# corelab-src/dacapo

Hardware: AMD Instinct MI355X
Metric: NTT/s (NTT-equivalents over one run() of the ResNet HEVM program, nt=2^14) (higher is better)
Workload: dtype u64; 1 GPU; ResNet-20 (SiLU) HEVM program traced from the reference's examples/benchmarks/ResNet.py with its resnet20.silu.model weights, nt=2^14 slots, N=2^15, 14 x 60-bit primes (SEAL_HEVM.cpp:39-53); one independent ciphertext stream per GPU; streams_per_gpu=1, parallelism=replicas x1 (no collective in the op path)

## Files before the change

### dacapo_amd/csrc/batch_ops.hip

```cpp
#include <stdlib.h>

#include "galois.hpp"
#include "plan.hpp"

namespace dacapo {

constexpr int kBT = 256;

__global__ __launch_bounds__(kBT) void b_tensor_kernel(const MulItem *__restrict__ items, u64 *__restrict__ target, int ell,
                                                        size_t N, const DModulus *__restrict__ mods)
{
    const int i = blockIdx.y, b = blockIdx.z;
    const MulItem it = items[b];
    const DModulus m = mods[i];
    const size_t k = ((size_t)blockIdx.x * kBT + threadIdx.x) * 2;
    const u64x2 a0 = *reinterpret_cast<const u64x2 *>(it.a.limb(0, i, N) + k), a1 = *reinterpret_cast<const u64x2 *>(it.a.limb(1, i, N) + k);
    const u64x2 b0 = *reinterpret_cast<const u64x2 *>(it.b.limb(0, i, N) + k), b1 = *reinterpret_cast<const u64x2 *>(it.b.limb(1, i, N) + k);
    u64x2 c0, c1, c2;
#pragma unroll
    for (int e = 0; e < 2; e++) {
        c0[e] = mulmod(a0[e], b0[e], m);
        Acc128 acc;
        acc.clear();
        acc.mac(a0[e], b1[e]);
        acc.mac(a1[e], b0[e]);
        c1[e] = acc.reduce(m);
        c2[e] = mulmod(a1[e], b1[e], m);
    }
    *reinterpret_cast<u64x2 *>(it.dst.limb(0, i, N) + k) = c0;
    *reinterpret_cast<u64x2 *>(it.dst.limb(1, i, N) + k) = c1;
    const size_t o = ((size_t)b * ell + i) * N + k;
    *reinterpret_cast<u64x2 *>(target + o) = c2;
}

template <int MODE>
__global__ __launch_bounds__(kBT) void b_ks_mac_kernel(u64 *__restrict__ acc, const u64 *__restrict__ ext,
                                                        const u64 *__restrict__ target, const KsItem *__restrict__ items,
                                                        const u64 *__restrict__ shared_key, int ell, int K, size_t N, int logN,
                                                        const DModulus *__restrict__ mods)
{
    const int m = blockIdx.y, b = blockIdx.z, sp = K - 1;
    const int pm = (m == ell) ? sp : m;
    const DModulus M = mods[pm];
    const u64 *key = MODE == 0 ? items[b].key : shared_key;
    const u64 *tg = MODE == 0 ? nullptr : target + (size_t)b * ell * N;
    const u64 *ex = ext + (size_t)b * ell * ell * N;
    const size_t k = ((size_t)blockIdx.x * kBT + threadIdx.x) * 2;
    Acc128 a0[2], a1[2];
    u64 r0[2] = { 0, 0 }, r1[2] = { 0, 0 };
#pragma unroll
    for (int e = 0; e < 2; e++) a0[e].clear(), a1[e].clear();
    for (int j = 0; j < ell; j++) {
        u64x2 x;
        if (j == m && MODE == 0) {
            const u32 g = galois_idx((u32)k, items[b].elt, logN);
            const u64x2 v = *reinterpret_cast<const u64x2 *>(items[b].src.limb(1, j, N) + (g & ~1u));
            x = (g & 1u) ? u64x2{ v.y, v.x } : v;
        } else {
            const u64 *op = (j == m) ? tg + (size_t)j * N : ex + ((size_t)j * ell + (m < j ? m : m - 1)) * N;
            x = *reinterpret_cast<const u64x2 *>(op + k);
        }
        const u64x2 y0 = *reinterpret_cast<const u64x2 *>(key + (((size_t)j * 2 + 0) * K + pm) * N + k);
        const u64x2 y1 = *reinterpret_cast<const u64x2 *>(key + (((size_t)j * 2 + 1) * K + pm) * N + k);
#pragma unroll
        for (int e = 0; e < 2; e++) {
            a0[e].mac(x[e], y0[e]);
            a1[e].mac(x[e], y1[e]);
        }
        if ((j & 15) == 15) {
#pragma unroll
            for (int e = 0; e < 2; e++) {
                r0[e] = addmod(r0[e], a0[e].reduce(M), M.q);
                r1[e] = addmod(r1[e], a1[e].reduce(M), M.q);
                a0[e].clear(), a1[e].clear();
            }
        }
    }
    u64x2 o0, o1;
#pragma unroll
    for (int e = 0; e < 2; e++) {
        o0[e] = addmod(r0[e], a0[e].reduce(M), M.q);
        o1[e] = addmod(r1[e], a1[e].reduce(M), M.q);
    }
    u64 *ac = acc + (size_t)b * 2 * (ell + 1) * N;
    *reinterpret_cast<u64x2 *>(ac + ((size_t)0 * (ell + 1) + m) * N + k) = o0;
    *reinterpret_cast<u64x2 *>(ac + ((size_t)1 * (ell + 1) + m) * N + k) = o1;
}

static bool fuse_mac() { return option(OPT_KS_FUSE_MAC) != 0; }
static long big_threshold() { return (long)option(OPT_KS_BIG_TILES); }
static long fuse_mac_threshold() { return (long)option(OPT_KS_FUSE_MAC_TILES); }

bool chain_fusion_supported() { return fuse_mac() && fuse_mac_threshold() == (1L << 40); }

template <int MODE>
static void b_ks_tail(Context &c, const BatchWs &w, u64 *digits, const KsItem *items, const void *final_items, const u64 *shared_key, int B,
                      int ell, hipStream_t s, const Handoff &h)
{
    const size_t N = c.N;
    const int K = c.K, sp = K - 1;
    const long tiles = (long)(N >> 10) * B * ell * ell;
    const bool big = tiles >= big_threshold(), fused_mac = fuse_mac() && tiles < fuse_mac_threshold();
    if (big) {
        launch_ntt_cols_inv(c, digits, (long)N, B * ell, nullptr, 0, ell, s);
        f_ks_lift_fcols(c, digits, w.ext, B, ell, s);
    } else
        f_ks_icols_lift_fcols(c, digits, w.ext, B, ell, s);
    u64 *acc_last = w.acc + (size_t)ell * N;
    const long acc_ps = (long)(ell + 1) * (long)N;
    if (!fused_mac) {
        launch_ntt_rows_fwd(c, w.ext, (long)N, B * ell * ell, c.ks_prime_idx(ell), 0, ell * ell, s);
        DC_LAUNCH(b_ks_mac_kernel<MODE>, dim3((unsigned)(N / (2 * kBT)), ell + 1, B), dim3(kBT), 0, s, w.acc, w.ext, w.target, items,
                           shared_key, ell, K, N, c.logN, c.d_mods);
        f_irows_strided(c, acc_last, acc_ps, sp, 1, acc_last, acc_ps, 2 * B, s);
    } else
        f_ks_frows_mac(c, MODE, w.ext, MODE == 1 ? nullptr : w.target, MODE == 1 ? reinterpret_cast<const KsItem *>(final_items) : items,
                       shared_key, w.acc, B, ell, s, MODE == 0);
    if (big) {
        launch_ntt_cols_inv(c, acc_last, acc_ps, 2 * B, nullptr, sp, 1, s);
        f_dr_lift_fcols(c, acc_last, acc_ps, w.tmp, 2 * B, ell, sp, s);
    } else
        f_dr_icols_lift_fcols(c, acc_last, acc_ps, w.tmp, 2 * B, ell, sp, s);
    f_frows_final(c, (MODE == 1 && fused_mac) ? 4 : MODE, w.tmp, final_items, w.acc, 2 * B, ell, sp, s, RsItem{}, nullptr, nullptr, h,
                  MODE == 0 && fused_mac);
}

void b_rotate_hops(Context &c, const BatchWs &w, const KsItem *d_items, int B, int ell, hipStream_t s, const Handoff &h, int unique)
{
    if (c.hybrid()) {
        hyb_rotate_hops(c, w, d_items, B, ell, s, unique);
        return;
    }
    f_irows_rot_c1(c, d_items, ell, w.digits, B, s);
    b_ks_tail<0>(c, w, w.digits, d_items, d_items, nullptr, B, ell, s, h);
}

void b_mul_relin(Context &c, const BatchWs &w, const MulItem *d_items, const u64 *relin_key, int B, int ell, hipStream_t s, const Handoff &h)
{
    if (c.hybrid()) {
        hyb_mul_relin(c, w, d_items, relin_key, B, ell, s);
        return;
    }
    const size_t N = c.N;
    const bool fused_mac = fuse_mac() && (long)(N >> 10) * B * ell * ell < fuse_mac_threshold();
    u64 *digits = w.digits;
    if (h.in)
        digits = const_cast<u64 *>(h.in);
    else if (!fused_mac) {
        DC_LAUNCH(b_tensor_kernel, dim3((unsigned)(N / (2 * kBT)), ell, B), dim3(kBT), 0, s, d_items, w.target, ell, N, c.d_mods);
        f_irows_strided(c, w.target, (long)N, 0, ell, w.digits, (long)N, B * ell, s);
    } else
        f_irows_tensor_c2(c, d_items, ell, w.digits, B, s);
    b_ks_tail<1>(c, w, digits, nullptr, d_items, relin_key, B, ell, s, h);
}

bool mul_relin_rescale_fused(const Context &c, int B, int ell)
{
    const long tiles = (long)(c.N >> 10) * B * ell * ell;
    return !c.hybrid() && ell >= 2 && fuse_mac() && tiles < fuse_mac_threshold() && tiles < big_threshold();
}

void b_mul_relin_rescale(Context &c, const BatchWs &w, const MulRsItem *d_items, const u64 *relin_key, int B, int ell, hipStream_t s, const Handoff &h)
{
    if (!mul_relin_rescale_fused(c, B, ell)) {
        fprintf(stderr, "[dacapo_amd] b_mul_relin_rescale: no folded form for %d items at level %d under this context / these launch options "
                        "(run b_mul_relin and b_rescale)\n", B, ell);
        abort();
    }
    const u64 *digits = h.in;
    if (!digits) {
        f_irows_tensor_c2_rs(c, d_items, ell, w.digits, B, s);
        digits = w.digits;
    }
    f_ks_icols_lift_fcols(c, digits, w.ext, B, ell, s);
    f_ks_frows_mac_rs(c, w.ext, d_items, relin_key, w.acc, B, ell, s);
    f_dr2_icols_lift_fcols(c, w.acc, d_items, w.tmp, B, ell, s);
    f_frows_fold_final(c, w.tmp, d_items, w.acc, B, ell, s, h);
}

void b_rescale(Context &c, const BatchWs &w, const RsItem *d_items, int B, int ell, hipStream_t s, const SumSrc *d_srcs, const Handoff &h)
{
    const int l = ell - 1;
    const u64 *last = w.digits;
    if (h.in)
        last = h.in;
    else
        f_irows_rs_last(c, d_items, d_srcs, l, w.digits, B, s);
    f_dr_icols_lift_fcols(c, last, (long)c.N, w.tmp, 2 * B, l, l, s);
    f_frows_final(c, 2, w.tmp, d_items, nullptr, 2 * B, l, l, s, RsItem{}, nullptr, d_srcs, h);
}

__global__ __launch_bounds__(kBT) void b_fill_const_kernel(u64 *__restrict__ out, const u64 *__restrict__ residues, size_t N)
{
    const size_t k = ((size_t)blockIdx.x * kBT + threadIdx.x) * 2;
    const u64 r = residues[blockIdx.y];
    *reinterpret_cast<u64x2 *>(out + (size_t)blockIdx.y * N + k) = u64x2{ r, r };
}
void fill_const_plain(Context &c, u64 *out, const u64 *d_residues, int ell, hipStream_t s)
{
    DC_LAUNCH(b_fill_const_kernel, dim3((unsigned)(c.N / (2 * kBT)), (unsigned)ell), dim3(kBT), 0, s, out, d_residues, c.N);
}

void rescale_fused(Context &c, const Workspace &w, CtView dst, CtView src, int ell, const u64 *plain, hipStream_t s)
{
    const int l = ell - 1;
    u64 *last = w.ks_digits;
    f_irows_rs_single(c, src, l, last, s);
    f_dr_icols_lift_fcols(c, last, (long)c.N, w.ks_tmp, 2, l, l, s);
    f_frows_final(c, 3, w.ks_tmp, nullptr, nullptr, 2, l, l, s, RsItem{ src, dst, 0, 0, nullptr, nullptr }, plain);
}

template <int OP>
__global__ __launch_bounds__(kBT) void b_ew_kernel(const EwItem *__restrict__ items, int polys, int b_polys, size_t N,
                                                    const DModulus *__restrict__ mods)
{
    const int i = blockIdx.y, p = blockIdx.z % polys, b = blockIdx.z / polys;
    const EwItem it = items[b];
// ... 275 lines not shown
```

### dacapo_amd/csrc/c_api.hip

```cpp
#include "../../include/dacapo_ckks.h"

#include <algorithm>
#include <vector>

#include "kernels.hpp"
#include "plan.hpp"

using namespace dacapo;

#include "c_api_types.hpp"

static inline hipStream_t S(void *s) { return (hipStream_t)s; }
static inline CtView V(const uint64_t *p, long stride) { return CtView{ const_cast<u64 *>(p), stride }; }

namespace {
constexpr int kItemSlots = 64;
constexpr size_t kItemBytes = 128;
static_assert(sizeof(KsItem) <= kItemBytes && sizeof(MulItem) <= kItemBytes && sizeof(RsItem) <= kItemBytes && sizeof(MulRsItem) <= kItemBytes, "item slot too small");
constexpr int kConstSlotWords = 64;
void *item_slot(dc_context *ctx, const void *host_item, size_t bytes, hipStream_t s)
{
    if (!ctx->item_ring) DC_HIP_CHECK(hipMalloc(&ctx->item_ring, kItemSlots * kItemBytes));
    char *slot = static_cast<char *>(ctx->item_ring) + (size_t)(ctx->item_next++ % kItemSlots) * kItemBytes;
    DC_HIP_CHECK(hipMemcpyAsync(slot, host_item, bytes, hipMemcpyHostToDevice, s));
// ... 182 lines not shown
{
    launch_add_plain(*ctx->c, V(dst, dst_stride), V(a, a_stride), plain, ell, S(stream));
}
void dc_ct_mul_plain(dc_context *ctx, uint64_t *dst, long dst_stride, const uint64_t *a, long a_stride, const uint64_t *plain,
                     int ell, void *stream)
{
    launch_ew(*ctx->c, EwOp::Mul, V(dst, dst_stride), V(a, a_stride), V(plain, 0), 2, 1, ell, S(stream));
}
void dc_ct_mul_relin(dc_context *ctx, uint64_t *dst, long dst_stride, const uint64_t *a, long a_stride, const uint64_t *b,
                     long b_stride, const uint64_t *relin_key, int ell, void *stream)
{
    if (overlaps(dst, a) || overlaps(dst, b)) {
        mul_relin(*ctx->c, ctx->c->ws0, V(dst, dst_stride), V(a, a_stride), V(b, b_stride), relin_key, ell, S(stream));
        return;
    }
    const MulItem it{ V(a, a_stride), V(b, b_stride), V(dst, dst_stride) };
    const MulItem *d = static_cast<const MulItem *>(item_slot(ctx, &it, sizeof(it), S(stream)));
    b_mul_relin(*ctx->c, batch_ws(ctx->c->ws0), d, relin_key, 1, ell, S(stream));
}
void dc_ct_mul_relin_rescale(dc_context *ctx, uint64_t *dst, long dst_stride, const uint64_t *a, long a_stride, const uint64_t *b,
                             long b_stride, const uint64_t *relin_key, const uint64_t *add_plain, const uint64_t *mul_const, int ell,
                             void *stream)
{
    Context &c = *ctx->c;
    hipStream_t s = S(stream);
    if (c.hybrid()) {
        fprintf(stderr, "[dacapo_amd] dc_ct_mul_relin_rescale: this context switches keys with grouped digits, whose mod-down is an approximate base "
                        "conversion; the call is for SEAL-layout keys (use dc_ct_mul_relin and dc_ct_rescale)\n");
        abort();
    }
    if (ell < 2 || ell > c.max_level() || ell > kConstSlotWords) {
        fprintf(stderr, "[dacapo_amd] dc_ct_mul_relin_rescale: level %d (2..%d)\n", ell, std::min(c.max_level(), kConstSlotWords));
        abort();
    }
    const size_t N = c.N;
    const u64 *d_consts = nullptr;
    if (mul_const) {
        if (!ctx->fold_consts) DC_HIP_CHECK(hipMalloc(&ctx->fold_consts, (size_t)kItemSlots * kConstSlotWords * sizeof(u64)));
        u64 *slot = ctx->fold_consts + (size_t)(ctx->item_next % kItemSlots) * kConstSlotWords;
        DC_HIP_CHECK(hipMemcpyAsync(slot, mul_const, (size_t)ell * sizeof(u64), hipMemcpyHostToDevice, s));
        d_consts = slot;
    }
    const bool fused = mul_relin_rescale_fused(c, 1, ell), alias = overlaps(dst, a) || overlaps(dst, b);
    if (!fused || alias) {
        const size_t need = (size_t)3 * ell * N * sizeof(u64);
        if (need > ctx->fold_tmp_cap) {
            if (ctx->fold_tmp) DC_HIP_CHECK(hipFree(ctx->fold_tmp));
            ctx->fold_tmp = nullptr;
            DC_HIP_CHECK(hipMalloc(&ctx->fold_tmp, need));
            ctx->fold_tmp_cap = need;
        }
    }
    if (fused) {
        const CtView out = alias ? CtView{ ctx->fold_tmp, (long)(ell - 1) * (long)N } : V(dst, dst_stride);
        MulRsItem it;
        it.a = V(a, a_stride), it.b = V(b, b_stride), it.dst = out;
        it.add = add_plain, it.mul = d_consts, it.mul_stride = 1;
        const MulRsItem *d = static_cast<const MulRsItem *>(item_slot(ctx, &it, sizeof(it), s));
        b_mul_relin_rescale(c, batch_ws(c.ws0), d, relin_key, 1, ell, s);
        if (alias) launch_ew(c, EwOp::Copy, V(dst, dst_stride), out, out, 2, 2, ell - 1, s);
        return;
    }
    const CtView prod{ ctx->fold_tmp, (long)ell * (long)N };
    u64 *mul_plain = nullptr;
    if (d_consts) {
        mul_plain = ctx->fold_tmp + (size_t)2 * ell * N;
        fill_const_plain(c, mul_plain, d_consts, ell, s);
    }
    const MulItem mi{ V(a, a_stride), V(b, b_stride), prod };
    b_mul_relin(c, batch_ws(c.ws0), static_cast<const MulItem *>(item_slot(ctx, &mi, sizeof(mi), s)), relin_key, 1, ell, s);
    const RsItem ri{ prod, V(dst, dst_stride), 0, 0, add_plain, mul_plain };
    b_rescale(c, batch_ws(c.ws0), static_cast<const RsItem *>(item_slot(ctx, &ri, sizeof(ri), s)), 1, ell, s);
}
void dc_ct_rotate_hop(dc_context *ctx, uint64_t *dst, long dst_stride, const uint64_t *src, long src_stride,
                      uint32_t galois_elt, const uint64_t *galois_key, int ell, void *stream)
{
    if (overlaps(dst, src)) {
        rotate_hop(*ctx->c, ctx->c->ws0, V(dst, dst_stride), V(src, src_stride), galois_elt, galois_key, ell, S(stream));
        return;
    }
    const KsItem it{ V(src, src_stride), V(dst, dst_stride), galois_key, galois_elt, 0 };
    const KsItem *d = static_cast<const KsItem *>(item_slot(ctx, &it, sizeof(it), S(stream)));
    b_rotate_hops(*ctx->c, batch_ws(ctx->c->ws0), d, 1, ell, S(stream));
}
void dc_ct_rotate_hoisted(dc_context *ctx, uint64_t *const *dsts, long dst_stride, const uint64_t *src, long src_stride,
                          const uint32_t *galois_elts, const uint64_t *const *galois_keys, int count, int ell, void *stream)
{
    const size_t B = (size_t)count;
    const KsItem *d = hoist_items(ctx, "dc_ct_rotate_hoisted", ", where dc_ct_rotate_hop already takes the digits before the automorphism", "hops",
                                  count, ell, B, S(stream), [&](std::vector<KsItem> &h) {
                                      for (size_t b = 0; b < B; b++)
                                          h.push_back(KsItem{ V(src, src_stride), V(dsts[b], dst_stride), galois_keys[b], galois_elts[b], 0 });
                                      h.push_back(KsItem{ V(src, src_stride), V(src, src_stride), nullptr, 1u, 0 });
                                      return (size_t)0;
                                  });
    Context &c = *ctx->c;
    const BatchWs w{ c.ws0.ct_tmp, c.ws0.ks_digits, c.ws0.ks_ext, ctx->hoist_acc, ctx->hoist_tmp };
    hoist_rotate_hops(c, w, d, d + B, count, 1, ell, S(stream));
}
void dc_ct_rotate_sum_hoisted(dc_context *ctx, uint64_t *dst, long dst_stride, const uint64_t *const *srcs, long src_stride,
                              const uint32_t *galois_elts, const uint64_t *const *galois_keys, const uint64_t *const *plains,
                              const uint64_t *const *plains_sp, int count, int ell, void *stream)
{
    const size_t B = (size_t)count;
    size_t U = 0;
    const KsItem *d = hoist_items(ctx, "dc_ct_rotate_sum_hoisted", " (ks_special > 1)", "members", count, ell, 1, S(stream), [&](std::vector<KsItem> &h) {
        std::vector<size_t> order(B);
        for (size_t b = 0; b < B; b++) order[b] = b;
        std::stable_sort(order.begin(), order.end(), [&](size_t x, size_t y) { return srcs[x] < srcs[y]; });
        std::vector<KsItem> sources;
        for (size_t b : order) {
            const u64 *pl = plains ? plains[b] : nullptr, *psp = plains_sp ? plains_sp[b] : nullptr;
            if ((pl == nullptr) != (psp == nullptr)) {
                fprintf(stderr, "[dacapo_amd] dc_ct_rotate_sum_hoisted: member %zu has one of plains / plains_sp only\n", b);
                abort();
            }
            const CtView sv = V(srcs[b], src_stride);
            if (sources.empty() || sources.back().src.p != sv.p) sources.push_back(KsItem{ sv, sv, nullptr, 1u, 0 });
            h.push_back(KsItem{ sv, V(dst, dst_stride), galois_keys[b], galois_elts[b], (u32)(sources.size() - 1), pl, psp });
        }
        h.push_back(KsItem{ V(dst, dst_stride), V(dst, dst_stride), nullptr, 0u, (u32)B });
        h.insert(h.end(), sources.begin(), sources.end());
        return U = sources.size();
    });
    const BatchWs w{ nullptr, ctx->hoist_digits, ctx->hoist_ext, ctx->hoist_acc, ctx->hoist_tmp };
    hoist_rotate_sum(*ctx->c, w, d, d + B + 1, count, (int)U, d + B, 1, ell, S(stream));
}
void dc_ct_rescale(dc_context *ctx, uint64_t *dst, long dst_stride, const uint64_t *src, long src_stride, int ell, void *stream)
{
    const RsItem it{ V(src, src_stride), V(dst, dst_stride), 0, 0, nullptr, nullptr };
    const RsItem *d = static_cast<const RsItem *>(item_slot(ctx, &it, sizeof(it), S(stream)));
    b_rescale(*ctx->c, batch_ws(ctx->c->ws0), d, 1, ell, S(stream));
}
void dc_ct_modswitch(dc_context *ctx, uint64_t *dst, long dst_stride, const uint64_t *src, long src_stride, int ell, int down,
                     void *stream)
{
    if (down <= 0 || (dst == src && dst_stride == src_stride)) return;
    launch_ew(*ctx->c, EwOp::Copy, V(dst, dst_stride), V(src, src_stride), V(src, src_stride), 2, 2, ell - down, S(stream));
}

void dc_keyswitch(dc_context *ctx, uint64_t *out, long out_stride, const uint64_t *base0, const uint64_t *base1,
                  const uint64_t *target, const uint64_t *key, int ell, void *stream)
{
    keyswitch(*ctx->c, ctx->c->ws0, V(out, out_stride), base0, base1, target, key, ell, S(stream));
}
void dc_galois_ntt(dc_context *ctx, uint64_t *dst, long dst_stride, const uint64_t *src, long src_stride, uint32_t galois_elt,
                   int polys, int ell, void *stream)
{
    launch_galois(*ctx->c, V(dst, dst_stride), V(src, src_stride), galois_elt, polys, ell, S(stream));
}
void dc_poly_mul(dc_context *ctx, uint64_t *dst, const uint64_t *a, const uint64_t *b, int ell, void *stream)
{
    launch_ew(*ctx->c, EwOp::Mul, V(dst, 0), V(a, 0), V(b, 0), 1, 1, ell, S(stream));
}
void dc_poly_add(dc_context *ctx, uint64_t *dst, const uint64_t *a, const uint64_t *b, int ell, void *stream)
{
    launch_ew(*ctx->c, EwOp::Add, V(dst, 0), V(a, 0), V(b, 0), 1, 1, ell, S(stream));
}

uint32_t dc_galois_elt_from_step(const dc_context *ctx, int step)
{
    const uint32_t n = (uint32_t)ctx->c->N, m = 2 * n;
    if (step == 0) return m - 1;
    const uint32_t pos = (uint32_t)(step < 0 ? -step : step);
    if (pos >= (n >> 1)) return 0;
    uint32_t e = step < 0 ? (n >> 1) - pos : pos;
// ... 10 lines not shown
```

### dacapo_amd/csrc/fused_ks.hip

```cpp
#include "ks_mac.hpp"

namespace dacapo {

struct SrcStrided {
    const u64 *base;
    long stride;
    int prime_base, period;
    __device__ int prime(int z) const { return prime_base + z % period; }
    __device__ u64 load(int z, int g, int) const { return base[(long)z * stride + g]; }
};
template <int E>
__device__ __forceinline__ void rs_operand(u64 (&v)[E], const int (&g)[E], const RsItem &it, const SumSrc *__restrict__ srcs, int p, int i,
                                           size_t N, const DModulus &M)
{
    if (it.count == 0) {
        const u64 *x = it.src.limb(p, i, N);
#pragma unroll
        for (int j = 0; j < E; j++) v[j] = x[g[j]];
    } else {
        u64 s[E];
        Acc128 a[E];
#pragma unroll
        for (int j = 0; j < E; j++) s[j] = 0, a[j].clear();
        int n_plain = 0, n_prod = 0;
// ... 252 lines not shown
        const u64 k2 = inv_last[(size_t)L * Kp + i];
        u64 k3 = mulmod(inv_last[(size_t)sp * Kp + i], k2, Mi);
        if (mul) k3 = mulmod(mul[(long)i * mul_stride], k3, Mi);
        u64 y[E];
#pragma unroll
        for (int r = 0; r < E; r++) {
            const u64 t = recanon(rho[r], Mi) + neg_half_p, w = recanon(u[r], Mi) + neg_half_l;
            Acc128 a;
            a.clear();
            a.mac(t >= qi ? t - qi : t, k3);
            a.mac(w >= qi ? w - qi : w, k2);
            y[r] = a.reduce(Mi);
        }
        __syncthreads();
        ntt_tile_fcols<K, LOGE, false, true, false>(
            y, Mi, tw + ((size_t)i << logN), tw2 ? tw2 + ((size_t)i << (K + 1)) : nullptr, logN, blockIdx.x, nold, [=](int g, u64 v) { out[g] = v; }, lds);
    }
}

template <int K, int LOGE>
__global__ __launch_bounds__(kTileThreads) void f_ks_lift_fcols_kernel(const u64 *__restrict__ digits, u64 *__restrict__ ext, int ell,
                                                                        int sp, const DModulus *__restrict__ mods,
                                                                        const u64 *__restrict__ tw, int logN, const u64 *__restrict__ tw2)
{
    __shared__ __attribute__((aligned(16))) u64 lds[TileGeo<LOGE>::LDS_ELEMS];
    const int z = blockIdx.y, e = z % ell, dj = z / ell, j = dj % ell;
    const size_t N = (size_t)1 << logN;
    const u64 *in = digits + (size_t)dj * N;
    u64 *out = ext + (size_t)z * N;
    const int pm = ks_other_prime(j, e, ell, sp);
    const DModulus Mm = mods[pm];
    u64 x[1 << LOGE];
    ntt_tile_fcols<K, LOGE, false, false, false>(
        x, Mm, tw + ((size_t)pm << logN), tw2 ? tw2 + ((size_t)pm << (K + 1)) : nullptr, logN, blockIdx.x,
        [=](int g) {
            return recanon(in[g], Mm);
        },
        [=](int g, u64 v) { out[g] = v; }, lds);
}

template <int K, int LOGE>
__global__ __launch_bounds__(kTileThreads) void f_dr_lift_fcols_kernel(const u64 *__restrict__ last, long last_stride,
                                                                        u64 *__restrict__ tmp, int cnt, int l, int Kp,
                                                                        const DModulus *__restrict__ mods,
                                                                        const u64 *__restrict__ half_mod, const u64 *__restrict__ tw,
                                                                        int logN, const u64 *__restrict__ tw2)
{
    __shared__ __attribute__((aligned(16))) u64 lds[TileGeo<LOGE>::LDS_ELEMS];
    const int z = blockIdx.y, i = z % cnt, bp = z / cnt;
    const size_t N = (size_t)1 << logN;
    const u64 *in = last + (long)bp * last_stride;
    u64 *out = tmp + (size_t)z * N;
    const DModulus Mi = mods[i];
    const u64 ql = mods[l].q, qi = Mi.q, half = ql >> 1;
    const u64 neg_half = qi - half_mod[(size_t)l * Kp + i];
    u64 x[1 << LOGE];
    ntt_tile_fcols<K, LOGE, false, false, false>(
        x, Mi, tw + ((size_t)i << logN), tw2 ? tw2 + ((size_t)i << (K + 1)) : nullptr, logN, blockIdx.x,
        [=](int g) {
            u64 y = in[g] + half;
            y = y >= ql ? y - ql : y;
            y = recanon(y, Mi);
            y += neg_half;
            return y >= qi ? y - qi : y;
        },
        [=](int g, u64 v) { out[g] = v; }, lds);
}

template <int K, int LOGE, int MODE>
__global__ __launch_bounds__(kTileThreads) void f_frows_final_kernel(const u64 *__restrict__ tmp, const void *__restrict__ items_,
                                                                      RsItem single, const u64 *__restrict__ plain,
                                                                      const SumSrc *__restrict__ srcs,
                                                                      const u64 *__restrict__ acc, int cnt, int l, int Kp,
                                                                      const DModulus *__restrict__ mods,
                                                                      const u64 *__restrict__ inv_last, const u64 *__restrict__ tw,
                                                                      int logN, int base_folded)
{
    __shared__ __attribute__((aligned(16))) u64 lds[TileGeo<LOGE>::LDS_ELEMS];
    const int z = blockIdx.y, i = z % cnt, bp = z / cnt, b = bp >> 1, p = bp & 1;
    const size_t N = (size_t)1 << logN;
    const DModulus M = mods[i];
    const u64 inv = inv_last[(size_t)l * Kp + i];
    const u64 *in = tmp + (size_t)z * N;
    if (MODE == 0 && base_folded) {
        constexpr int E = 1 << LOGE;
        const KsItem it = reinterpret_cast<const KsItem *>(items_)[b];
        const u64 *x = acc + (((size_t)bp) * (cnt + 1) + i) * N;
        u64 *o = it.dst.limb(p, i, N);
        u64 v[E];
        auto nost = [](int, u64) {};
        ntt_tile_x<K, LOGE, false, false, true, false, true>(v, M, tw + ((size_t)i << logN), logN, blockIdx.x, [=](int gi) { return in[gi]; }, nost, lds);
        const int g0 = tile_gidx<K, LOGE, false>(num_passes<LOGE>(K) - 1, logN, blockIdx.x, 0);
#pragma unroll
        for (int j = 0; j < E; j += 2) {
            const u64x2 a = *reinterpret_cast<const u64x2 *>(x + g0 + j);
            u64x2 r;
            r.x = mulmod(submod(a.x, v[j], M.q), inv, M), r.y = mulmod(submod(a.y, v[j + 1], M.q), inv, M);
            *reinterpret_cast<u64x2 *>(o + g0 + j) = r;
        }
    } else if (MODE == 0) {
        const KsItem it = reinterpret_cast<const KsItem *>(items_)[b];
        const u64 *x = acc + (((size_t)bp) * (cnt + 1) + i) * N;
        const u64 *c0 = it.src.limb(0, i, N);
        u64 *o = it.dst.limb(p, i, N);
        ntt_tile<K, LOGE, false, false, true>(
            M, tw + ((size_t)i << logN), logN, blockIdx.x, [=](int g) { return in[g]; },
            [=](int g, u64 v) {
                const u64 base = p == 0 ? c0[galois_idx((u32)g, it.elt, logN)] : 0;
                o[g] = addmod(base, mulmod(submod(x[g], v, M.q), inv, M), M.q);
            },
            lds);
    } else if (MODE == 1) {
        const MulItem it = reinterpret_cast<const MulItem *>(items_)[b];
        const u64 *x = acc + (((size_t)bp) * (cnt + 1) + i) * N;
        u64 *o = it.dst.limb(p, i, N);
        ntt_tile<K, LOGE, false, false, true>(
            M, tw + ((size_t)i << logN), logN, blockIdx.x, [=](int g) { return in[g]; },
            [=](int g, u64 v) { o[g] = addmod(o[g], mulmod(submod(x[g], v, M.q), inv, M), M.q); }, lds);
    } else if (MODE == 4) {
        const MulItem it = reinterpret_cast<const MulItem *>(items_)[b];
        const u64 *x = acc + (((size_t)bp) * (cnt + 1) + i) * N;
        const u64 *a0 = it.a.limb(0, i, N), *a1 = it.a.limb(1, i, N), *b0 = it.b.limb(0, i, N), *b1 = it.b.limb(1, i, N);
        u64 *o = it.dst.limb(p, i, N);
        constexpr int E = 1 << LOGE;
        u64 v[E], base[E];
        int g[E];
        auto nost = [](int, u64) {};
        ntt_tile_x<K, LOGE, false, false, true, false, true>(v, M, tw + ((size_t)i << logN), logN, blockIdx.x,
                                                             [=](int gi) { return in[gi]; }, nost, lds);
#pragma unroll
        for (int j = 0; j < E; j++) g[j] = tile_gidx<K, LOGE, false>(num_passes<LOGE>(K) - 1, logN, blockIdx.x, j);
        if (p == 0) {
#pragma unroll
            for (int j = 0; j < E; j++) base[j] = mulmod(a0[g[j]], b0[g[j]], M);
        } else {
#pragma unroll
            for (int j = 0; j < E; j++) {
                Acc128 t;
                t.clear();
                t.mac(a0[g[j]], b1[g[j]]);
                t.mac(a1[g[j]], b0[g[j]]);
                base[j] = t.reduce(M);
            }
        }
#pragma unroll
        for (int j = 0; j < E; j++) o[g[j]] = addmod(base[j], mulmod(submod(x[g[j]], v[j], M.q), inv, M), M.q);
    } else if (MODE == 3) {
        const u64 *x = single.src.limb(p, i, N);
        u64 *o = single.dst.limb(p, i, N);
        const u64 *pl = (plain && p == 0) ? plain + (size_t)i * N : nullptr;
        ntt_tile<K, LOGE, false, false, true>(
            M, tw + ((size_t)i << logN), logN, blockIdx.x, [=](int g) { return in[g]; },
            [=](int g, u64 v) {
                const u64 r = mulmod(submod(x[g], v, M.q), inv, M);
                o[g] = pl ? addmod(r, pl[g], M.q) : r;
            },
            lds);
    } else {
        const RsItem it = reinterpret_cast<const RsItem *>(items_)[b];
        u64 *o = it.dst.limb(p, i, N);
        constexpr int E = 1 << LOGE;
        u64 x[E], op[E];
        int g[E];
        auto nost = [](int, u64) {};
        ntt_tile_x<K, LOGE, false, false, true, false, true>(x, M, tw + ((size_t)i << logN), logN, blockIdx.x,
                                                             [=](int gi) { return in[gi]; }, nost, lds);
#pragma unroll
        for (int j = 0; j < E; j++) g[j] = tile_gidx<K, LOGE, false>(num_passes<LOGE>(K) - 1, logN, blockIdx.x, j);
        rs_operand<E>(op, g, it, srcs, p, i, N, M);
#pragma unroll
        for (int j = 0; j < E; j++) o[g[j]] = mulmod(submod(op[j], x[j], M.q), inv, M);
    }
}

template <int K, int LOGE, int MODE>
__device__ __forceinline__ void final_value(u64 (&v)[1 << LOGE], const int (&g)[1 << LOGE], const u64 *__restrict__ in, const void *__restrict__ items_,
                                            const SumSrc *__restrict__ srcs, const u64 *__restrict__ acc, int b, int p, int i, int cnt,
                                            const DModulus &M, u64 inv, const u64 *__restrict__ tw, int logN, u64 *__restrict__ lds,
                                            bool base_folded = false)
{
    constexpr int E = 1 << LOGE;
    const size_t N = (size_t)1 << logN;
    auto nost = [](int, u64) {};
    u64 x[E];
    ntt_tile_x<K, LOGE, false, false, true, false, true>(x, M, tw + ((size_t)i << logN), logN, blockIdx.x, [=](int gi) { return in[gi]; }, nost, lds);
    if (MODE == 4) {
        const MulItem it = reinterpret_cast<const MulItem *>(items_)[b];
        const u64 *ac = acc + (((size_t)(b * 2 + p)) * (cnt + 1) + i) * N;
        const u64 *a0 = it.a.limb(0, i, N), *a1 = it.a.limb(1, i, N), *b0 = it.b.limb(0, i, N), *b1 = it.b.limb(1, i, N);
        u64 *o = it.dst.limb(p, i, N);
#pragma unroll
        for (int j = 0; j < E; j++) {
            u64 base;
            if (p == 0)
                base = mulmod(a0[g[j]], b0[g[j]], M);
            else {
                Acc128 t;
                t.clear();
                t.mac(a0[g[j]], b1[g[j]]);
                t.mac(a1[g[j]], b0[g[j]]);
                base = t.reduce(M);
            }
            v[j] = addmod(base, mulmod(submod(ac[g[j]], x[j], M.q), inv, M), M.q);
            o[g[j]] = v[j];
        }
    } else if (MODE == 0) {
        const KsItem it = reinterpret_cast<const KsItem *>(items_)[b];
        const u64 *ac = acc + (((size_t)(b * 2 + p)) * (cnt + 1) + i) * N;
        const u64 *c0 = it.src.limb(0, i, N);
        u64 *o = it.dst.limb(p, i, N);
#pragma unroll
        for (int j = 0; j < E; j++) {
            const u64 base = (p == 0 && !base_folded) ? c0[galois_idx((u32)g[j], it.elt, logN)] : 0;
            v[j] = addmod(base, mulmod(submod(ac[g[j]], x[j], M.q), inv, M), M.q);
            o[g[j]] = v[j];
        }
    } else {
        const RsItem it = reinterpret_cast<const RsItem *>(items_)[b];
        u64 *o = it.dst.limb(p, i, N);
        u64 op[E];
        rs_operand<E>(op, g, it, srcs, p, i, N, M);
#pragma unroll
        for (int j = 0; j < E; j++) {
            v[j] = mulmod(submod(op[j], x[j], M.q), inv, M);
            o[g[j]] = v[j];
        }
    }
}

template <int K, int LOGE, int MODE, int CONT>
__global__ __launch_bounds__(kTileThreads) void f_frows_final_cont_kernel(const u64 *__restrict__ tmp, const void *__restrict__ items_,
                                                                           const SumSrc *__restrict__ srcs, const u64 *__restrict__ acc, int cnt,
                                                                           int l, int Kp, const DModulus *__restrict__ mods,
                                                                           const u64 *__restrict__ inv_last, const u64 *__restrict__ tw,
                                                                           const u64 *__restrict__ itw, int logN, Handoff h, int base_folded)
{
    __shared__ __attribute__((aligned(16))) u64 lds[TileGeo<LOGE>::LDS_ELEMS];
    constexpr int E = 1 << LOGE, NP = num_passes<LOGE>(K);
    const size_t N = (size_t)1 << logN;
    int g[E];
#pragma unroll
    for (int j = 0; j < E; j++) g[j] = tile_gidx<K, LOGE, false>(NP - 1, logN, blockIdx.x, j);
    auto nold = [](int) -> u64 { return 0; };
    if (CONT == CONT_BOOT) {
        const int z = blockIdx.y, i = z % cnt, b = z / cnt;
        const DModulus M = mods[i];
        const u64 inv = inv_last[(size_t)l * Kp + i];
        u64 v0[E], v1[E];
        final_value<K, LOGE, MODE>(v0, g, tmp + ((size_t)(b * 2 + 0) * cnt + i) * N, items_, srcs, acc, b, 0, i, cnt, M, inv, tw, logN, lds, base_folded != 0);
        __syncthreads();
        final_value<K, LOGE, MODE>(v1, g, tmp + ((size_t)(b * 2 + 1) * cnt + i) * N, items_, srcs, acc, b, 1, i, cnt, M, inv, tw, logN, lds, base_folded != 0);
        const u64 *sk = h.sk + (size_t)i * N;
#pragma unroll
        for (int j = 0; j < E; j++) v0[j] = addmod(v0[j], mulmod(v1[j], sk[g[j]], M), M.q);
        __syncthreads();
        u64 *o = h.out + (size_t)z * N;
        ntt_tile_x<K, LOGE, false, true, false, true, false>(v0, M, itw + ((size_t)i << logN), logN, blockIdx.x, nold, [=](int gi, u64 v) { o[gi] = v; }, lds);
    } else {
        const int z = blockIdx.y, i = z % cnt, bp = z / cnt, b = bp >> 1, p = bp & 1;
        const DModulus M = mods[i];
        const u64 inv = inv_last[(size_t)l * Kp + i];
        u64 v[E];
        final_value<K, LOGE, MODE>(v, g, tmp + (size_t)z * N, items_, srcs, acc, b, p, i, cnt, M, inv, tw, logN, lds, base_folded != 0);
        if (CONT == CONT_RS) {
            if (i != cnt - 1) return;
            const RsItem cit = h.rs_items[b];
            if (cit.add && p == 0) {
                const u64 *w = cit.add + (size_t)i * N;
#pragma unroll
                for (int j = 0; j < E; j++) v[j] = addmod(v[j], w[g[j]], M.q);
            }
            if (cit.mul) {
                const u64 *w = cit.mul + (size_t)i * N;
#pragma unroll
                for (int j = 0; j < E; j++) v[j] = mulmod(v[j], w[g[j]], M);
            }
            __syncthreads();
            u64 *o = h.out + (size_t)bp * N;
            ntt_tile_x<K, LOGE, false, true, false, true, false>(v, M, itw + ((size_t)i << logN), logN, blockIdx.x, nold, [=](int gi, u64 y) { o[gi] = y; }, lds);
        } else {
            if (p != 1) return;
            const CtView other = h.other[b];
            if (other.p) {
                const u64 *o1 = other.limb(1, i, N);
#pragma unroll
                for (int j = 0; j < E; j++) v[j] = mulmod(v[j], o1[g[j]], M);
            } else {
#pragma unroll
                for (int j = 0; j < E; j++) v[j] = mulmod(v[j], v[j], M);
            }
            __syncthreads();
            u64 *o = h.out + ((size_t)b * cnt + i) * N;
            ntt_tile_x<K, LOGE, false, true, false, true, false>(v, M, itw + ((size_t)i << logN), logN, blockIdx.x, nold, [=](int gi, u64 y) { o[gi] = y; }, lds);
        }
    }
}

// ... 427 lines not shown
            DC_K_SWITCH(c.k1, DC_LAUNCH((KERNEL<KK, LE, true>), grid, dim3(kTileThreads), 0, s, __VA_ARGS__))                    \
        } else if (le == 2) {                                                                                                             \
            constexpr int LE = 2;                                                                                                         \
            const dim3 grid((unsigned)(c.N >> TileGeo<LE>::LOG), (unsigned)(sources));                                                    \
            DC_K_SWITCH(c.k1, DC_LAUNCH((KERNEL<KK, LE, true>), grid, dim3(kTileThreads), 0, s, __VA_ARGS__))                    \
        } else {                                                                                                                          \
            constexpr int LE = 3;                                                                                                         \
            const dim3 grid((unsigned)(c.N >> TileGeo<LE>::LOG), (unsigned)(sources));                                                    \
            DC_K_SWITCH(c.k1, DC_LAUNCH((KERNEL<KK, LE, true>), grid, dim3(kTileThreads), 0, s, __VA_ARGS__))                    \
        }                                                                                                                                 \
    }

void f_ks_icols_lift_fcols(const Context &c, const u64 *digits, u64 *ext, int B, int ell, hipStream_t s)
{
    DC_MERGED_LAUNCH(B * ell * ell, B * ell, ell, f_ks_icols_lift_fcols_kernel, digits, ext, ell, c.K - 1, c.d_mods, c.d_tw, c.d_itw, c.logN, c.twc2())
}

void f_dr_icols_lift_fcols(const Context &c, const u64 *last, long last_stride, u64 *tmp, int polys, int cnt, int l, hipStream_t s)
{
    DC_MERGED_LAUNCH(polys * cnt, polys, cnt, f_dr_icols_lift_fcols_kernel, last, last_stride, tmp, cnt, l, c.K, c.d_mods, c.d_half_mod, c.d_tw,
                     c.d_itw, c.logN, c.twc2())
}

void f_dr2_icols_lift_fcols(const Context &c, const u64 *acc, const MulRsItem *items, u64 *tmp, int B, int ell, hipStream_t s)
{
    DC_MERGED_LAUNCH(2 * B * (ell - 1), 2 * B, ell - 1, f_dr2_icols_lift_fcols_kernel, acc, items, tmp, ell, c.K, c.d_mods, c.d_half_mod, c.d_inv_last,
                     c.d_tw, c.d_itw, c.logN, c.twc2())
}
#undef DC_MERGED_LAUNCH

void f_frows_fold_final(const Context &c, const u64 *tmp, const MulRsItem *items, const u64 *acc, int B, int ell, hipStream_t s, const Handoff &h)
{
    const int cnt = ell - 1, groups = h.cont == CONT_BOOT ? B : 2 * B;
#define DC_FOLD(CT)                                                                                                                    \
    DC_GEO_SWITCH(c.k2, groups * cnt, DC_LAUNCH((f_frows_fold_final_kernel<KK, LE, CT>), grid, dim3(kTileThreads), 0, s, tmp, items, acc, ell, c.K, \
                                                         c.d_mods, c.d_inv_last, c.d_tw, c.d_itw, c.logN, h))
    switch (h.cont) {
    case CONT_NONE: DC_FOLD(CONT_NONE); break;
    case CONT_MUL: DC_FOLD(CONT_MUL); break;
    case CONT_BOOT: DC_FOLD(CONT_BOOT); break;
    default: fprintf(stderr, "[dacapo_amd] f_frows_fold_final: no continuation kernel for consumer kind %d\n", h.cont); abort();
    }
#undef DC_FOLD
}

void f_ks_lift_fcols(const Context &c, const u64 *digits, u64 *ext, int B, int ell, hipStream_t s)
{
    if ((c.k1 == 7 || c.k1 == 8) && use_wide_tiles(c.N, (long)B * ell * ell) && !use_small_tiles(c.N, (long)B * ell * ell)) {
        constexpr int LE = 4;
        const dim3 grid((unsigned)(c.N >> TileGeo<LE>::LOG), (unsigned)(B * ell * ell));
        if (c.k1 == 7)
            DC_LAUNCH((f_ks_lift_fcols_kernel<7, LE>), grid, dim3(kTileThreads), 0, s, digits, ext, ell, c.K - 1, c.d_mods, c.d_tw, c.logN, c.twc2());
        else
            DC_LAUNCH((f_ks_lift_fcols_kernel<8, LE>), grid, dim3(kTileThreads), 0, s, digits, ext, ell, c.K - 1, c.d_mods, c.d_tw, c.logN, c.twc2());
        return;
    }
    DC_GEO_SWITCH(c.k1, B * ell * ell, DC_LAUNCH((f_ks_lift_fcols_kernel<KK, LE>), grid, dim3(kTileThreads), 0, s, digits, ext, ell,
                                                          c.K - 1, c.d_mods, c.d_tw, c.logN, c.twc2()));
}

void f_dr_lift_fcols(const Context &c, const u64 *last, long last_stride, u64 *tmp, int polys, int cnt, int l, hipStream_t s)
{
    DC_GEO_SWITCH(c.k1, polys * cnt, DC_LAUNCH((f_dr_lift_fcols_kernel<KK, LE>), grid, dim3(kTileThreads), 0, s, last, last_stride,
                                                        tmp, cnt, l, c.K, c.d_mods, c.d_half_mod, c.d_tw, c.logN, c.twc2()));
}

void f_frows_final(const Context &c, int mode, const u64 *tmp, const void *items, const u64 *acc, int polys, int cnt, int l,
                   hipStream_t s, RsItem single, const u64 *plain, const SumSrc *srcs, const Handoff &h, bool base_folded)
{
    const int folded = base_folded ? 1 : 0;
    if (h.cont != CONT_NONE) {
        const int groups = h.cont == CONT_BOOT ? polys / 2 : polys;
#define DC_CONT(MD, CT)                                                                                                                \
    DC_GEO_SWITCH(c.k2, groups * cnt, DC_LAUNCH((f_frows_final_cont_kernel<KK, LE, MD, CT>), grid, dim3(kTileThreads), 0, s, tmp, items, \
                                                         srcs, acc, cnt, l, c.K, c.d_mods, c.d_inv_last, c.d_tw, c.d_itw, c.logN, h, folded))
        if (mode == 4 && h.cont == CONT_RS) {
            DC_CONT(4, CONT_RS);
        } else if (mode == 2 && h.cont == CONT_MUL) {
            DC_CONT(2, CONT_MUL);
        } else if (mode == 2 && h.cont == CONT_BOOT) {
            DC_CONT(2, CONT_BOOT);
        } else if (mode == 0 && h.cont == CONT_BOOT) {
            DC_CONT(0, CONT_BOOT);
        } else {
            fprintf(stderr, "[dacapo_amd] f_frows_final: no continuation kernel for mode %d -> consumer kind %d\n", mode, h.cont);
            abort();
        }
#undef DC_CONT
        return;
    }
#define DC_FINAL(MD)                                                                                                                   \
    DC_GEO_SWITCH(c.k2, polys * cnt, DC_LAUNCH((f_frows_final_kernel<KK, LE, MD>), grid, dim3(kTileThreads), 0, s, tmp, items, single, \
                                                        plain, srcs, acc, cnt, l, c.K, c.d_mods, c.d_inv_last, c.d_tw, c.logN, folded))
    switch (mode) {
    case 0: DC_FINAL(0); break;
    case 1: DC_FINAL(1); break;
    case 2: DC_FINAL(2); break;
    case 4: DC_FINAL(4); break;
    default: DC_FINAL(3); break;
    }
#undef DC_FINAL
}

}
```

### dacapo_amd/csrc/hevm_vm.hip

```cpp
#include "hevm_vm.hpp"

#include "../../include/dacapo_ckks.h"
#include "c_api_types.hpp"
#include "chacha.hpp"
#include "seal_serial.hpp"

#include <math.h>
#include <string.h>
#include <sys/random.h>

#include <algorithm>
#include <cmath>
#include <chrono>
#include <fstream>
#include <iostream>

namespace dacapo {

constexpr int kVmThreads = 256;

constexpr int kRngCoefs = 8;

__device__ __forceinline__ int rng_cbd(u64 w)
{
// ... 312 lines not shown
    }
}

void HostEncoder::decode(std::vector<std::complex<double>> &v, double *out) const
{
    for (size_t m = 1, gap = N >> 1; m < N; m <<= 1, gap >>= 1)
        for (size_t i = 0; i < m; i++) {
            const std::complex<double> r = root_[m + i];
            std::complex<double> *x = v.data() + 2 * i * gap, *y = x + gap;
            for (size_t j = 0; j < gap; j++) {
                const std::complex<double> a = x[j], b = y[j] * r;
                x[j] = a + b;
                y[j] = a - b;
            }
        }
    for (size_t i = 0; i < slots; i++) out[i] = v[slot_map_[i]].real();
}

RngKeys rng_keys_from_os()
{
    RngKeys k;
    unsigned char buf[sizeof(RngKeys)];
    size_t got = 0;
    while (got < sizeof(buf)) {
        const ssize_t r = getrandom(buf + got, sizeof(buf) - got, 0);
        if (r <= 0) {
            fprintf(stderr, "[dacapo_amd] getrandom() failed: no cryptographic randomness available, refusing to generate keys or encrypt\n");
            abort();
        }
        got += (size_t)r;
    }
    memcpy(&k, buf, sizeof(k));
    return k;
}


static u64 *dalloc(size_t elems)
{
    u64 *p = nullptr;
    DC_HIP_CHECK(vm_malloc(&p, elems * sizeof(u64)));
    return p;
}

void HEVM::init_context(int logN, int K, const u64 *primes, int dir_ksp, int dir_alpha)
{
    int ndev = 0;
    if (hipGetDeviceCount(&ndev) != hipSuccess || ndev == 0) {
        fprintf(stderr, "[dacapo_amd] no HIP device: the HEVM runtime has no CPU fallback\n");
        abort();
    }
    int ksp = std::max(1, (int)option(OPT_KS_SPECIAL));
    int alpha = option(OPT_KS_ALPHA) > 0 ? (int)option(OPT_KS_ALPHA) : ksp;
    if (dir_ksp > 0) {
        if ((ksp != 1 || alpha != 1) && (ksp != dir_ksp || alpha != dir_alpha)) {
            fprintf(stderr, "[dacapo_amd] the key directory was written with ks_special = %d, ks_alpha = %d; options ask for %d / %d\n", dir_ksp,
                    dir_alpha, ksp, alpha);
            abort();
        }
        ksp = dir_ksp, alpha = dir_alpha;
    }
    ks_hoist = option(OPT_KS_HOIST) != 0;
    if (ks_hoist && (ksp > 1 || alpha > 1)) {
        fprintf(stderr, "[dacapo_amd] option ks_hoist = 1 is for SEAL-layout keys (ks_special = 1); with ks_special = %d, ks_alpha = %d key switching uses "
                        "grouped digits, which already shares a source's decomposition among its hops\n", ksp, alpha);
        abort();
    }
    ks_lazy = (int)option(OPT_KS_LAZY_SUM);
    if (ks_lazy && (ksp > 1 || alpha > 1)) {
        fprintf(stderr, "[dacapo_amd] option ks_lazy_sum = %d is for SEAL-layout keys (ks_special = 1); with ks_special = %d, ks_alpha = %d the lazy sums "
                        "of grouped-digit key switching are options hyb_lazy_sum / hyb_double_hoist\n", ks_lazy, ksp, alpha);
        abort();
    }
    if (ks_lazy && !ks_hoist) {
        fprintf(stderr, "[dacapo_amd] option ks_lazy_sum = %d needs ks_hoist = 1: a lazy sum is defined on digits taken before the automorphism "
                        "(ks_hoist = 0 here)\n", ks_lazy);
        abort();
    }
    ks_fold_rescale = option(OPT_KS_FOLD_RESCALE) != 0;
    if (ks_fold_rescale && (ksp > 1 || alpha > 1)) {
        fprintf(stderr, "[dacapo_amd] option ks_fold_rescale = 1 is for SEAL-layout keys (ks_special = 1); with ks_special = %d, ks_alpha = %d the mod-down "
                        "is an approximate base conversion, and dividing by P q in one exact pass does not reproduce it\n", ksp, alpha);
        abort();
    }
    const int bits = (int)option(OPT_PRIME_BITS);
    ctx.reset(new Context(logN, K, bits, primes, ksp, alpha));
    ctx->ensure_scratch();
    encoder.reset(new HostEncoder(logN));
    use_plan = option(OPT_PLAN) != 0;
    plan_graph = option(OPT_PLAN_GRAPH) != 0;
    plan_dag = option(OPT_PLAN_GRAPH) == 2;
    plan_lanes = option(OPT_PLAN_LANES) >= 2 ? 2 : 1;
    host_encoder = option(OPT_HOST_ENCODER) != 0;
    fold_rescale_into_boot = option(OPT_FOLD_RESCALE_BOOT) != 0;
    lazy_sums = option(OPT_HYB_LAZY_SUM) != 0;
    double_hoist = (lazy_sums && option(OPT_HYB_DOUBLE_HOIST) != 0) || ks_lazy == 2;
    max_batch = std::max(1, (int)option(OPT_MAX_BATCH));
    chain_fusion = option(OPT_CHAIN_FUSION) != 0;
    secret_weight = (int)option(OPT_SECRET_HW);
    boot_secret_weight = (int)option(OPT_BOOT_SECRET_HW);
    rot_compose = option(OPT_ROT_COMPOSE) != 0;
    online_encode = option(OPT_ONLINE_ENCODE) != 0 && use_plan && !host_encoder;
    lanes.resize(1);
    DC_HIP_CHECK(hipStreamCreateWithFlags(&lanes[0].stream, hipStreamNonBlocking));
    lanes[0].ws = ctx->ws0;
    lanes[0].boot_plain.d = dalloc((size_t)ctx->max_level() * ctx->N);
    lanes[0].boot_plain.level = ctx->max_level();
    DC_HIP_CHECK(vm_malloc(&d_epoch, 8));
    DC_HIP_CHECK(hipMemset(d_epoch, 0, 8));
    cur = 0;
}

void HEVM::gen_kswitch_key(u64 *key, const u64 *new_key, u64 key_id) { gen_kswitch_key_in(*ctx, key, keys.sk, new_key, key_id); }

void HEVM::gen_kswitch_key_in(Context &c, u64 *key, const u64 *key_sk, const u64 *new_key, u64 key_id)
{
    const size_t N = c.N;
    const int K = c.K;
    const dim3 gu((unsigned)(N / (kRngCoefs * kVmThreads)), (unsigned)K), gs((unsigned)(N / (kRngCoefs * kVmThreads))),
        g2((unsigned)(N / (2 * kVmThreads)), (unsigned)K);
    const int L = c.max_level();
    for (int j = 0; j < c.key_digits(); j++) {
        u64 *c0 = key + (size_t)j * 2 * K * N, *c1 = c0 + (size_t)K * N;
        const u64 object = key_id * 64 + (u64)j;
        DC_LAUNCH(sample_uniform_kernel, gu, dim3(kVmThreads), 0, S(), c1, N, rng.pub, object, (u32)RNG_KSK_A, c.d_mods);
        DC_LAUNCH(sample_small_kernel, gs, dim3(kVmThreads), 0, S(), c0, N, K, 1, rng.secret, object, (u32)RNG_KSK_E, c.d_mods);
        launch_ntt(c, false, c0, (long)N, K, nullptr, 0, 0, S());
        const int lo = c.hybrid() ? j * c.alpha : j, hi = c.hybrid() ? std::min(lo + c.alpha, L) : j + 1;
        DC_LAUNCH(ezs_final_kernel, g2, dim3(kVmThreads), 0, S(), c0, c1, key_sk, new_key, lo, hi, c.d_pmod, N, c.d_mods);
    }
}

void HEVM::fill_sparse_secret(u64 *dst, int weight, u32 domain)
{
    const Context &c = *ctx;
    const size_t N = c.N;
    const int K = c.K;
    if (weight < 1 || (size_t)weight > N / 2) {
        fprintf(stderr, "[dacapo_amd] a sparse secret of weight %d is not sparse for N = %zu\n", weight, N);
        abort();
    }
    std::vector<int8_t> coef(N, 0);
    u64 w[8];
    int placed = 0;
    for (u64 blk = 0; placed < weight; blk++) {
        rng_words8(rng.secret, 0, blk, 0, 1, domain, w);
        for (int e = 0; e < 8 && placed < weight; e++) {
            const size_t idx = (size_t)((w[e] >> 8) % N);
            if (coef[idx]) continue;
            coef[idx] = (w[e] & 1) ? 1 : -1;
            placed++;
        }
    }
    std::vector<u64> h((size_t)K * N);
    for (int i = 0; i < K; i++)
        for (size_t k = 0; k < N; k++) h[(size_t)i * N + k] = coef[k] == 0 ? 0 : coef[k] > 0 ? 1 : c.primes[(size_t)i] - 1;
    DC_HIP_CHECK(hipMemcpyAsync(dst, h.data(), h.size() * 8, hipMemcpyHostToDevice, S()));
    DC_HIP_CHECK(hipStreamSynchronize(S()));
    explicit_bzero(h.data(), h.size() * sizeof(u64));
    explicit_bzero(coef.data(), coef.size());
    explicit_bzero(w, sizeof(w));
}

void HEVM::ensure_boot_context()
{
    if (bctx) return;
    const Context &c = *ctx;
// ... 1176 lines not shown
    f_irows_decrypt(c, src, keys.sk, ell, pt, S());
    launch_ntt_cols_inv(c, pt, (long)N, ell, nullptr, 0, 0, S());
    const CrtDev cd{ tb.inv, tb.mmod, tb.hmod, tb.hdig, tb.mdbl };
    DC_LAUNCH(reencode_kernel, dim3((unsigned)((N / 2 + kVmThreads) / kVmThreads)), dim3(kVmThreads), 0, S(), lohi,
                       lohi + N, pt, ell, N, c.d_mods, cd, new_scale / src_scale);
    Plain ptx{ lanes[cur].boot_plain.d, target_level, new_scale };
    DC_LAUNCH(lift_i128_kernel, dim3((unsigned)(N / kVmThreads), (unsigned)target_level), dim3(kVmThreads), 0, S(),
                       ptx.d, lohi, lohi + N, N, c.d_mods);
    launch_ntt(c, false, ptx.d, (long)N, target_level, nullptr, 0, 0, S());
    encrypt_plain(dst, ptx);
}

void HEVM::plan_zero_encrypt(int first, int B, int t, hipStream_t s)
{
    Context &c = *ctx;
    const size_t N = c.N;
    const int cnt = t + 1;
    if (!keys.pk) {
        fprintf(stderr, "[dacapo_amd] bootstrap: this VM has no public key\n");
        abort();
    }
    Plan &P = plan;
    DC_LAUNCH(sample_enc_batch_kernel, dim3((unsigned)(N / (kRngCoefs * kVmThreads)), (unsigned)(3 * B)), dim3(kVmThreads), 0, s,
                       P.boot_ue, N, cnt, rng.secret, ((u64)1 << 32) + (u64)first, c.d_mods, d_epoch);
    launch_ntt(c, false, P.boot_ue, (long)N, 3 * cnt * B, nullptr, 0, cnt, s);
    DC_LAUNCH(pk_encrypt_batch_kernel, dim3((unsigned)(N / (2 * kVmThreads)), (unsigned)cnt, (unsigned)(2 * B)), dim3(kVmThreads),
                       0, s, P.boot_tmp, keys.pk, (long)c.K * (long)N, P.boot_ue, cnt, N, c.d_mods);
    b_rescale(c, P.ws[0], P.d_boot_rs + first, B, cnt, s);
}

void HEVM::plan_boot_step(int first, int B, int ell, int t, int lane, hipStream_t s, const Handoff &h)
{
    Context &c = *ctx;
    const size_t N = c.N;
    if (!keys.sk) {
        fprintf(stderr, "[dacapo_amd] bootstrap: needs a full VM (secret + public key)\n");
        abort();
    }
    Plan &P = plan;
    const BootItem *items = P.d_boot + first;
    const CrtTables &tb = crt_tables(ell);
    const CrtDev cd{ tb.inv, tb.mmod, tb.hmod, tb.hdig, tb.mdbl };
    u64 *pt = P.boot_pt[lane], *ptx = P.boot_ptx[lane];
    if (h.in)
        pt = const_cast<u64 *>(h.in);
    else
        f_irows_decrypt_items(c, items, P.d_sum_srcs, keys.sk, ell, pt, B, s);
    launch_ntt_cols_inv(c, pt, (long)N, B * ell, nullptr, 0, ell, s);
    if (ell == 1)
        f_boot_reencode_fcols(c, pt, ptx, items, B, ell, t, cd, s);
    else {
        DC_LAUNCH(reencode_lift_batch_kernel, dim3((unsigned)((N / 2 + kVmThreads) / kVmThreads), (unsigned)B), dim3(kVmThreads), 0,
                           s, ptx, pt, items, ell, t, N, c.d_mods, cd);
        launch_ntt_cols_fwd(c, ptx, (long)N, B * t, nullptr, 0, t, s);
    }
    f_frows_boot_final(c, ptx, items, B, t, s);
}

void HEVM::dispatch(const WireOp &op)
{
    switch (op.opcode) {
    case 1: op_rotate(op.dst, op.lhs, (int16_t)op.rhs); break;
    case 2: op_negate(op.dst, op.lhs); break;
    case 3: op_rescale(op.dst, op.lhs); break;
    case 4: op_modswitch(op.dst, op.lhs, (int16_t)op.rhs); break;
    case 5: fprintf(stderr, "This VM does not support native upscale op\n"); abort();
    case 6: op_addcc(op.dst, op.lhs, op.rhs); break;
    case 7: op_addcp(op.dst, op.lhs, op.rhs); break;
    case 8: op_mulcc(op.dst, op.lhs, op.rhs); break;
    case 9: op_mulcp(op.dst, op.lhs, op.rhs); break;
    case 10: op_bootstrap(op.dst, op.lhs, op.rhs); break;
    case kOpConj: op_conj(op.dst, op.lhs); break;
    case kOpModRaise: op_modraise(op.dst, op.lhs, op.rhs); break;
    case kOpSetScale: op_setscale(op.dst, op.lhs, op.rhs); break;
    case kOpKeySwitch: op_keyswitch(op.dst, op.lhs, op.rhs); break;
    default: break;
    }
}

void HEVM::execute()
{
    memset(op_counts, 0, sizeof(op_counts));
    n_keyswitch = n_ntt = 0;
    n_hops = n_decomp = 0, n_fold = 0;
    t_bootstrap = 0.0;
    int i = (int)((header.hevm_header_size + config.config_body_length) / 8), j = 0;
    for (const WireOp &op : ops) {
        if (debug) {
            std::cout << std::endl;
            std::cout << std::oct << i++ << " " << std::dec << j++ << std::endl;
            std::cout << "opcode [" << op.opcode << "], dst [" << op.dst << "], lhs [" << op.lhs << "], rhs [" << op.rhs << "]"
                      << std::endl;
        }
        if (op.opcode <= 10) op_counts[op.opcode]++;
        if (op.opcode == 0 || (op.opcode > 10 && (op.opcode < kOpConj || op.opcode > kOpKeySwitch))) continue;
        dispatch(op);
    }
    bump_epoch(S());
}

void HEVM::run()
{
    if (use_plan && !debug) {
        run_plan();
        return;
    }
    if (streams != 1) {
        fprintf(stderr, "[dacapo_amd] several ciphertext streams need the batched plan (option plan = 1, no debug)\n");
        abort();
    }
    execute();
    DC_HIP_CHECK(hipStreamSynchronize(S()));
}

}

namespace dacapo {
thread_local VmAllocs *g_vm_allocs = nullptr;

void HEVM::destroy_device_state()
{
    (void)hipDeviceSynchronize();
    drop_plan_graph();
    for (Lane &ln : lanes)
        if (ln.stream) (void)hipStreamDestroy(ln.stream), ln.stream = nullptr;
    if (aux_stream) (void)hipStreamDestroy(aux_stream), aux_stream = nullptr;
    for (hipEvent_t e : plan.events) (void)hipEventDestroy(e);
    plan.events.clear();
    const std::vector<void *> live(allocs.live.begin(), allocs.live.end());
    allocs.live.clear();
    for (void *p : live) (void)hipFree(p);
}
}

using dacapo::HEVM;
static HEVM *V(void *vm)
{
    HEVM *h = static_cast<HEVM *>(vm);
    dacapo::g_vm_allocs = &h->allocs;
    return h;
}

static std::vector<char> slurp(const char *path)
{
    std::ifstream f(path, std::ios::in | std::ios::binary | std::ios::ate);
    if (!f) {
        fprintf(stderr, "[dacapo_amd] cannot open %s\n", path);
        abort();
    }
    std::vector<char> buf((size_t)f.tellg());
    f.seekg(0);
    f.read(buf.data(), (std::streamsize)buf.size());
    return buf;
}

static void env_params(int &logN, int &K)
{
    logN = (int)dacapo::option(dacapo::OPT_LOGN), K = (int)dacapo::option(dacapo::OPT_PRIMES);
}

extern "C" {

void *initFullVM(char *dir, bool device)
{
    (void)device;
    auto vm = new HEVM();
    vm->load_keys(dir, true, true, true);
// ... 215 lines not shown
    put_params(w, p);
    write_object_file(path, w.buf, (sio::Compr)compr_mode);
}
int hevm_seal_load_parms(const char *path, uint64_t *poly_modulus_degree, uint64_t *primes, int capacity)
{
    namespace sio = dacapo::sealio;
    const std::vector<uint8_t> file = sio::read_file(path);
    std::vector<uint8_t> owned;
    sio::Reader outer(file.data(), file.size(), path);
    sio::Reader m = open_object(outer, owned);
    const sio::Params p = get_params(m);
    if (p.scheme != sio::kSchemeCkks) m.fail("scheme is not CKKS");
    *poly_modulus_degree = p.N;
    for (size_t i = 0; i < p.primes.size() && (int)i < capacity; i++) primes[i] = p.primes[i];
    return (int)p.primes.size();
}
void hevm_seal_save_ciphertext(const char *path, int compr_mode, uint64_t poly_modulus_degree, const uint64_t *primes, int limbs, int size,
                               int is_ntt, double scale, const uint64_t *data)
{
    namespace sio = dacapo::sealio;
    sio::Writer w;
    sio::CtHeader h;
    h.id = sio::parms_id(poly_modulus_degree, primes, (size_t)limbs);
    h.is_ntt = is_ntt != 0, h.size = (uint64_t)size, h.N = poly_modulus_degree, h.limbs = (uint64_t)limbs, h.scale = scale;
    put_ciphertext(w, h, data);
    write_object_file(path, w.buf, (sio::Compr)compr_mode);
}
int64_t hevm_seal_load_ciphertext(const char *path, uint64_t *poly_modulus_degree, int *limbs, int *size, int *is_ntt, double *scale,
                                  uint64_t parms_id[4], uint64_t *data, uint64_t capacity)
{
    namespace sio = dacapo::sealio;
    const std::vector<uint8_t> file = sio::read_file(path);
    std::vector<uint8_t> owned;
    sio::Reader outer(file.data(), file.size(), path);
    sio::Reader m = open_object(outer, owned);
    const uint64_t *src = nullptr;
    const sio::CtHeader h = get_ciphertext(m, src);
    *poly_modulus_degree = h.N, *limbs = (int)h.limbs, *size = (int)h.size, *is_ntt = h.is_ntt ? 1 : 0, *scale = h.scale;
    memcpy(parms_id, h.id.data(), 32);
    const uint64_t words = h.size * h.N * h.limbs;
    if (data && words <= capacity) memcpy(data, src, (size_t)words * 8);
    return (int64_t)words;
}
int hevm_seal_zstd_available(void) { return dacapo::sealio::zstd_available() ? 1 : 0; }
void hevm_chacha20_block(const uint32_t key[8], uint64_t counter, uint64_t nonce, uint32_t out[16])
{
    dacapo::ChaChaKey k;
    memcpy(k.w, key, 32);
    uint32_t o[16];
    dacapo::chacha20_block(k, counter, nonce, o);
    memcpy(out, o, 64);
}
void hevm_chacha20_blocks_device(const uint32_t key[8], uint64_t counter, uint64_t nonce, int blocks, uint32_t *out_host)
{
    dacapo::ChaChaKey k;
    memcpy(k.w, key, 32);
    uint32_t *d = nullptr;
    DC_HIP_CHECK(hipMalloc(&d, (size_t)blocks * 64));
    DC_LAUNCH(dacapo::chacha_blocks_kernel, dim3((unsigned)((blocks + 63) / 64)), dim3(64), 0, 0, d, k, counter, nonce, blocks);
    DC_HIP_CHECK(hipMemcpy(out_host, d, (size_t)blocks * 64, hipMemcpyDeviceToHost));
    (void)hipFree(d);
}

void hevm_last_run_stats(void *vm, int64_t *op_counts, int64_t *keyswitches, int64_t *ntts)
{
    auto h = V(vm);
    if (op_counts) memcpy(op_counts, h->op_counts, sizeof(h->op_counts));
    if (keyswitches) *keyswitches = h->n_keyswitch;
    if (ntts) *ntts = h->n_ntt;
}

void hevm_last_run_hoist_stats(void *vm, int64_t *hops, int64_t *decompositions)
{
    auto h = V(vm);
    if (hops) *hops = h->n_hops;
    if (decompositions) *decompositions = h->n_decomp;
}

void hevm_last_run_fold_rescale_stats(void *vm, int64_t *pairs)
{
    if (pairs) *pairs = V(vm)->n_fold;
}

int64_t hevm_plan_lazy_groups(void *vm, int32_t *out, int64_t cap)
{
    auto h = V(vm);
    if (!h->plan.ready) return -1;
    std::vector<int32_t> flat;
    for (const auto &p : h->plan.pops)
        if (!p.dead && p.kind == HEVM::P_ROTSUM) {
            flat.push_back((int32_t)p.ops.size());
            flat.insert(flat.end(), p.ops.begin(), p.ops.end());
        }
    if (out && cap >= (int64_t)flat.size()) memcpy(out, flat.data(), flat.size() * sizeof(int32_t));
    return (int64_t)flat.size();
}

void hevm_destroy(void *vm)
{
    if (!vm) return;
    HEVM *h = V(vm);
    h->destroy_device_state();
    dacapo::g_vm_allocs = nullptr;
    delete static_cast<dc_context *>(h->ckks_handle);
    delete h;
}

}
```

### dacapo_amd/csrc/hevm_vm.hpp

```cpp
#pragma once
#include "wire_parse.hpp"
#include <complex>
#include <deque>
#include <map>
#include <set>
#include <memory>
#include <string>
#include <unordered_set>
#include <vector>

#include "../../include/hevm_abi.h"
#include "chacha.hpp"
#include "seal_serial.hpp"
#include "kernels.hpp"
#include "encoder.hpp"
#include "plan.hpp"

namespace dacapo {

struct VmAllocs {
    std::unordered_set<void *> live;
};
extern thread_local VmAllocs *g_vm_allocs;
template <class T>
// ... 49 lines not shown
    std::unique_ptr<Context> bctx;
    void ensure_boot_context();
    std::unique_ptr<HostEncoder> encoder;
    KeySet keys;
    bool debug = false;
    void *ckks_handle = nullptr;
    RngKeys rng;
    u64 enc_counter = 0;
    u64 *d_epoch = nullptr;

    struct Lane {
        hipStream_t stream = nullptr;
        Workspace ws;
        Plain boot_plain;
    };
    std::vector<Lane> lanes;
    int cur = 0;
    hipStream_t S() const { return lanes[cur].stream; }
    const Workspace &W() const { return lanes[cur].ws; }
    void execute();
    void dispatch(const WireOp &op);

    std::vector<std::vector<double>> buffer;
    EncTables enc_tables;
    std::vector<u64 *> plain_arenas;
    bool online_encode = false;
    struct OnlineEncode {
        double *d_consts = nullptr;
        size_t const_bytes = 0;
        std::map<int, EncItem> items;
    } online;
    bool host_encoder = false;
    void ensure_enc_tables();
    void preprocess_device();
    void free_plains();
    WireHeader header{};
    WireConfigBody config{};
    std::vector<WireOp> ops;
    std::vector<uint64_t> arg_scale, arg_level, res_scale, res_level, res_dst;
    std::deque<hevm_ctxt> ciphers;
    std::vector<Plain> plains;

    struct CrtTables {
        u64 *inv, *mmod, *hmod, *hdig;
        double *mdbl;
    };
    std::map<int, CrtTables> crt_;
    const CrtTables &crt_tables(int ell);

    enum PopKind { P_ROT, P_MULCC, P_RESCALE, P_SUM, P_NEG, P_MULP, P_ADDP, P_COPY, P_BOOT, P_MODRAISE, P_ROTSUM };
    static constexpr int kPopKinds = 11;
    struct Val {
        int level = 0;
        double scale = 1.0;
        int root = -1;
        int def_step = -1;
        int last_use = -1;
        int uses = 0;
        int def_pop = -1;
        u64 *buf = nullptr;
        bool external = false, pinned = false;
    };
    struct Pop {
        PopKind kind;
        int level = 0;
        int dst = -1;
        std::vector<int> srcs;
        std::vector<int> src_plain;
        u32 elt = 0;
        const u64 *key = nullptr;
        int plain = -1, target_level = 0;
        int rot = 0;
        int rs_add = -1, rs_mul = -1;
        bool rs_sum = false;
        int boot_drop = -1;
        double boot_src_scale = 0.0;
        bool dead = false;
        int wave = 0, step = -1;
        int op = -1;
        bool direct = false;
        std::vector<u32> elts;
        std::vector<const u64 *> keys;
        std::vector<int> ops;
        std::vector<int> plains;
    };
    struct Step {
        PopKind kind;
        int level = 0, first = 0, count = 0;
        int target = 0;
        int wave = 0, lane = 0;
        Handoff h;
        int fused_consumer = -1;
        bool fold_rs = false;
        int gfirst = 0, gcount = 0;
        int unique = 0;
        std::vector<const u64 *> reads, writes;
    };
    struct Plan {
        bool ready = false;
        std::vector<Val> vals;
        std::vector<Pop> pops;
        std::vector<Step> steps;
        std::vector<int> final_val;
        KsItem *d_ks = nullptr;
        MulItem *d_mul = nullptr;
        MulRsItem *d_mulrs = nullptr;
        RsItem *d_rs = nullptr;
        EwItem *d_ew = nullptr;
        SumItem *d_sum = nullptr;
        SumSrc *d_sum_srcs = nullptr;
        SumGroup *d_sumg = nullptr;
        SumGroupSrc *d_sumg_srcs = nullptr;
        CtView *d_cont_other = nullptr;
        struct EncGroup { int wave, level, first, count; u64 *out; };
        std::vector<EncGroup> enc_groups;
        EncItem *d_enc_items = nullptr;
        u64 *enc_arena = nullptr;
        double2 *enc_scratch = nullptr;
        int *d_enc_overflow = nullptr;
        size_t enc_arena_bytes = 0, enc_scratch_bytes = 0;
        std::vector<EwItem> h_ew;
        std::vector<u64 *> handoff_bufs;
        size_t n_fused = 0;
        BootItem *d_boot = nullptr;
        RsItem *d_boot_rs = nullptr;
        size_t zenc_bytes = 0;
        u64 *zenc = nullptr, *boot_ue = nullptr, *boot_tmp = nullptr, *boot_pt[2] = { nullptr, nullptr }, *boot_ptx[2] = { nullptr, nullptr };
        struct BootChunk { int first, count, target; };
        std::vector<BootChunk> boot_chunks;
        BatchWs ws[2];
        std::vector<hipEvent_t> events;
        std::vector<u64 *> pool;
        int64_t n_keyswitch = 0, n_ntt = 0;
        int64_t n_hops = 0, n_decomp = 0;
        int64_t n_fold = 0;
        size_t launches = 0, max_live = 0;
        hipGraph_t graph = nullptr;
        hipGraphExec_t graph_exec = nullptr;
    } plan;
    bool plan_graph = true;
    bool plan_dag = false;
    void capture_plan();
    bool capture_plan_dag();
    void issue_step(const Step &st, hipStream_t q);
    void drop_plan_graph();
    void issue_plan(hipStream_t s);
    bool use_plan = true;
    bool test_zero_enc = false;
    int max_batch = 64;
    std::vector<u64 *> home;
    int streams = 1, sel = 0;
    std::vector<u64 *> reg_base;
    void set_streams(int n);
    void select_stream(int s);
    void build_plan();
    void run_plan();
    void boot_item(CtView src, int src_level, double src_scale, hevm_ctxt &dst, int target_level);
    void plan_zero_encrypt(int first, int B, int t, hipStream_t s);
    void plan_boot_step(int first, int B, int ell, int t, int lane, hipStream_t s, const Handoff &h);
    bool rot_compose = false;
    std::vector<int> compose_rotation(int steps) const;
    mutable std::vector<int> rot_offsets;
    mutable std::set<int> rot_offset_set;
    mutable size_t rot_offsets_epoch = (size_t)-1;
    int boot_secret_weight = 0;
    int secret_weight = 0;
    bool ks_hoist = false;
    int ks_lazy = 0;
    bool ks_fold_rescale = false;
    KsItem *d_hoist_items = nullptr;
    void rotate_hop_vm(CtView dst, CtView src, u32 elt, const u64 *key, int ell);
    bool chain_fusion = true;
    hipStream_t aux_stream = nullptr;
    bool double_hoist = false;
    double *dh_consts = nullptr;
    std::map<int, EncItem> dh_items;
    void ensure_special_limbs(const std::vector<int> &plain_regs);
    bool lazy_sums = false;
    bool fold_rescale_into_boot = false;
    int plan_lanes = 2;
    void bump_epoch(hipStream_t s);

    int64_t op_counts[11] = { 0 };
    int64_t n_keyswitch = 0, n_ntt = 0;
    int64_t n_hops = 0, n_decomp = 0;
    int64_t n_fold = 0;
    double t_bootstrap = 0.0;

    VmAllocs allocs;
    HEVM() { g_vm_allocs = &allocs; }
    void destroy_device_state();
    size_t key_elems() const { return (size_t)ctx->key_digits() * 2 * ctx->K * ctx->N; }
    void init_context(int logN, int K, const u64 *primes, int dir_ksp = 0, int dir_alpha = 0);
    void generate_keys(const RngKeys &rng, bool secret, bool pub, bool eval);
    void gen_kswitch_key(u64 *key, const u64 *new_key, u64 key_id);
    void gen_kswitch_key_in(Context &c, u64 *key, const u64 *key_sk, const u64 *new_key, u64 key_id);
    void fill_sparse_secret(u64 *dst, int weight, u32 domain);
    void generate_boot_switch_keys();
    size_t swk_down_elems() const { return (size_t)2 * (1 + ctx->ksp) * ctx->N; }
    void add_galois_key(u32 elt);
    void save_keys(const std::string &dir);
    void load_keys(const std::string &dir, bool need_secret, bool need_public, bool need_eval);
    sealio::ParmsId parms_id_at(int limbs) const;
    sealio::ParmsId boot_parms_id() const { return sealio::parms_id(bctx->N, bctx->primes.data(), (size_t)bctx->K); }
    void save_ctxt(size_t reg, const std::string &path);
    void load_ctxt(size_t reg, const std::string &path);

    void load_constants(const void *data, size_t len);
    void load_program(const void *data, size_t len, bool header_only);
    void reset_res_dst();
    void preprocess();
    void encode_internal(Plain &dst, const double *src, size_t len, int level, int scale_bits);
    hevm_ctxt &reg(size_t i);
    void encrypt_plain(hevm_ctxt &dst, const Plain &pt);
    void encrypt(int64_t i, const double *dat, int len);
    void decrypt(int64_t i, double *out);
    void run();

    void op_rotate(int dst, int src, int offset);
    void op_negate(int dst, int src);
    void op_rescale(int dst, int src);
    void op_modswitch(int dst, int src, int down);
    void op_addcc(int dst, int lhs, int rhs);
    void op_addcp(int dst, int lhs, int rhs);
    void op_mulcc(int dst, int lhs, int rhs);
    void op_mulcp(int dst, int lhs, int rhs);
    void op_bootstrap(int dst, int src, int target_level);
    void op_conj(int dst, int src);
    void op_modraise(int dst, int src, int target);
    void op_setscale(int dst, int src, int const_idx);
    void op_keyswitch(int dst, int src, int which);
    std::vector<u32> rotate_hops(int steps) const;

    CtView view(const hevm_ctxt &c) const { return CtView{ c.data, (long)c.poly_stride }; }
};

}
```

### dacapo_amd/csrc/options.cpp

```cpp
#include "options.hpp"

#include "../../include/hevm_abi.h"

#include <stdio.h>
#include <stdlib.h>
#include <string.h>

namespace dacapo {

struct OptDef {
    const char *name;
    long long def;
};
static const OptDef kDefs[OPT_COUNT] = {
    { "logn", 15 },
    { "primes", 14 },
    { "prime_bits", 60 },
    { "ks_special", 1 },
    { "ks_alpha", 0 },
    { "secret_hw", 0 },
    { "boot_secret_hw", 0 },
    { "rot_compose", 0 },
    { "plan", 1 },
    { "plan_graph", 1 },
    { "plan_lanes", 2 },
    { "plan_aux_min_cost", 3 },
    { "max_batch", 64 },
    { "chain_fusion", 1 },
    { "host_encoder", 0 },
    { "online_encode", 0 },
    { "fold_rescale_boot", 0 },
    { "hyb_mfma", 1 },
    { "hyb_fuse", 2 },
    { "hyb_lazy_sum", 0 },
    { "hyb_double_hoist", 0 },
    { "ks_hoist", 0 },
    { "ks_lazy_sum", 0 },
    { "ks_fold_rescale", 0 },
    { "seal_compr", 0 },
    { "trace", 0 },
    { "step_profile", 0 },
    { "small_tile_wgs", -1 },
    { "tiny_tile_wgs", 2000 },
    { "wide_tile_wgs", 2048 },
    { "rows_prime_major", 16 },
    { "ntt_full_min_limbs", 768 },
    { "ntt_full_inv_min_limbs", 768 },
    { "ntt_full_persist", -1 },
    { "ntt_full_inv_persist", -1 },
    { "ntt_full_pairs", 1 },
    { "ntt_full_inv_pairs", 1 },
    { "cols_pairs", 1 },
    { "ks_merge_special_min_wgs", 2048 },
    { "ks_merge_lift_min_wgs", 1024 },
    { "ks_items_fast", 1 },
    { "ks_fuse_mac", 1 },
    { "ks_big_tiles", 4096 },
    { "ks_fuse_mac_tiles", 1LL << 40 },
    { "sum_pair_min_wgs", 1024 },
    { "sum_group_min_wgs", 2048 },
};

static long long g_val[OPT_COUNT];
static bool g_init = false;

static int find(const char *name, size_t len)
{
    for (int i = 0; i < OPT_COUNT; i++)
        if (strlen(kDefs[i].name) == len && !strncmp(kDefs[i].name, name, len)) return i;
    return -1;
}

static void unknown(const char *what, const char *name, size_t len)
{
    fprintf(stderr, "[dacapo_amd] %s: unknown option \"%.*s\"; known:", what, (int)len, name);
    for (int i = 0; i < OPT_COUNT; i++) fprintf(stderr, " %s", kDefs[i].name);
    fprintf(stderr, "\n");
    abort();
}

static long long parse_value(int opt, const char *v, size_t len)
{
    if (opt == OPT_SEAL_COMPR) {
        static const char *const names[] = { "none", "zlib", "zstd" };
        for (int k = 0; k < 3; k++)
            if (strlen(names[k]) == len && !strncmp(names[k], v, len)) return k;
    }
    char buf[32];
    char *end = nullptr;
    if (len == 0 || len >= sizeof buf) goto bad;
    memcpy(buf, v, len), buf[len] = 0;
    {
        const long long r = strtoll(buf, &end, 0);
        if (end != buf && *end == 0) return r;
    }
bad:
    fprintf(stderr, "[dacapo_amd] DACAPO_HEVM_OPTIONS: option \"%s\" needs an integer value%s, got \"%.*s\"\n", kDefs[opt].name,
            opt == OPT_SEAL_COMPR ? " (or none | zlib | zstd)" : "", (int)len, v);
    abort();
}

extern "C" char **environ;
static void warn_legacy_environment()
{
    for (char **e = environ; e && *e; e++) {
        if (strncmp(*e, "DACAPO_", 7) != 0) continue;
        if (!strncmp(*e, "DACAPO_HEVM_OPTIONS=", 20) || !strncmp(*e, "DACAPO_AMD_LIB=", 15) || !strncmp(*e, "DACAPO_FORCE_DIST=", 18) ||
            !strncmp(*e, "DACAPO_AMD_HOOKS=", 17))
            continue;
        const char *eq = strchr(*e, '=');
        fprintf(stderr, "[dacapo_amd] warning: environment variable %.*s is no longer read (round 4 replaced the per-knob variables); use "
                        "DACAPO_HEVM_OPTIONS=\"name=value,...\" or hevm_set_option() -- names: include/hevm_abi.h, csrc/options.hpp\n",
                eq ? (int)(eq - *e) : (int)strlen(*e), *e);
    }
}

static void init()
{
    if (g_init) return;
    g_init = true;
    for (int i = 0; i < OPT_COUNT; i++) g_val[i] = kDefs[i].def;
    warn_legacy_environment();
    const char *e = getenv("DACAPO_HEVM_OPTIONS");
    while (e && *e) {
        const char *end = strchr(e, ',');
        const size_t len = end ? (size_t)(end - e) : strlen(e);
        const char *eq = (const char *)memchr(e, '=', len);
        if (len) {
            if (!eq) unknown("DACAPO_HEVM_OPTIONS (expected name=value)", e, len);
            const int i = find(e, (size_t)(eq - e));
            if (i < 0) unknown("DACAPO_HEVM_OPTIONS", e, (size_t)(eq - e));
            g_val[i] = parse_value(i, eq + 1, len - (size_t)(eq + 1 - e));
        }
        e = end ? end + 1 : nullptr;
    }
}

long long option(Opt o)
{
    init();
    return g_val[o];
}

// ... 28 lines not shown
```

### dacapo_amd/csrc/options.hpp

```cpp
#pragma once

namespace dacapo {

enum Opt : int {
    OPT_LOGN,
    OPT_PRIMES,
    OPT_PRIME_BITS,
    OPT_KS_SPECIAL,
    OPT_KS_ALPHA,
    OPT_SECRET_HW,
    OPT_BOOT_SECRET_HW,
    OPT_ROT_COMPOSE,
    OPT_PLAN,
    OPT_PLAN_GRAPH,
    OPT_PLAN_LANES,
    OPT_PLAN_AUX_MIN_COST,
    OPT_MAX_BATCH,
    OPT_CHAIN_FUSION,
    OPT_HOST_ENCODER,
    OPT_ONLINE_ENCODE,
    OPT_FOLD_RESCALE_BOOT,
    OPT_HYB_MFMA,
    OPT_HYB_FUSE,
    OPT_HYB_LAZY_SUM,
    OPT_HYB_DOUBLE_HOIST,
    OPT_KS_HOIST,
    OPT_KS_LAZY_SUM,
    OPT_KS_FOLD_RESCALE,
    OPT_SEAL_COMPR,
    OPT_TRACE,
    OPT_STEP_PROFILE,
    OPT_SMALL_TILE_WGS,
    OPT_TINY_TILE_WGS,
    OPT_WIDE_TILE_WGS,
    OPT_ROWS_PRIME_MAJOR,
    OPT_NTT_FULL_MIN_LIMBS,
    OPT_NTT_FULL_INV_MIN_LIMBS,
    OPT_NTT_FULL_PERSIST,
    OPT_NTT_FULL_INV_PERSIST,
    OPT_NTT_FULL_PAIRS,
    OPT_NTT_FULL_INV_PAIRS,
    OPT_COLS_PAIRS,
    OPT_KS_MERGE_SPECIAL_MIN_WGS,
    OPT_KS_MERGE_LIFT_MIN_WGS,
    OPT_KS_ITEMS_FAST,
    OPT_KS_FUSE_MAC,
    OPT_KS_BIG_TILES,
    OPT_KS_FUSE_MAC_TILES,
    OPT_SUM_PAIR_MIN_WGS,
    OPT_SUM_GROUP_MIN_WGS,
    OPT_COUNT
};

long long option(Opt o);

}
```

### dacapo_amd/csrc/plan.hpp

```cpp
#pragma once
#include "crt_device.hpp"
#include "kernels.hpp"

namespace dacapo {

struct KsItem {
    CtView src, dst;
    const u64 *key;
    u32 elt;
    u32 slot;
    const u64 *plain = nullptr, *plain_sp = nullptr;
};
struct MulItem {
    CtView a, b, dst;
};
struct MulRsItem : MulItem {
    const u64 *add = nullptr;
    const u64 *mul = nullptr;
    long mul_stride = 0;
};
struct RsItem {
    CtView src, dst;
    int first = 0, count = 0;
    const u64 *add = nullptr;
    const u64 *mul = nullptr;
};
struct EwItem {
    CtView dst, a, b;
};
struct SumSrc {
    CtView v;
    const u64 *plain;
};
struct SumItem {
    CtView dst;
    int first, count;
};

constexpr int kSumGroup = 8;
struct SumGroupSrc {
    CtView v;
    const u64 *plain[kSumGroup];
};
struct SumGroup {
    CtView dst[kSumGroup];
    int first, count, items;
};
__host__ __device__ inline const u64 *sum_add_only() { return reinterpret_cast<const u64 *>((uintptr_t)8); }

struct BootItem {
    CtView src, dst;
    const u64 *zenc;
    double ratio;
    int first = 0, count = 0;
    const u64 *add = nullptr, *mul = nullptr;
};

enum ContKind : int {
    CONT_NONE = 0,
    CONT_RS = 1,
    CONT_MUL = 2,
    CONT_BOOT = 3,
};
struct Handoff {
    int cont = CONT_NONE;
    u64 *out = nullptr;
    const CtView *other = nullptr;
    const struct RsItem *rs_items = nullptr;
    const u64 *sk = nullptr;
    const u64 *in = nullptr;
};

struct BatchWs {
    u64 *target = nullptr;
    u64 *digits = nullptr;
    u64 *ext = nullptr;
    u64 *acc = nullptr;
    u64 *tmp = nullptr;
};

void b_rotate_hops(Context &c, const BatchWs &w, const KsItem *d_items, int B, int ell, hipStream_t s, const Handoff &h = Handoff{}, int unique = 0);
void b_mul_relin(Context &c, const BatchWs &w, const MulItem *d_items, const u64 *relin_key, int B, int ell, hipStream_t s,
                 const Handoff &h = Handoff{});
bool mul_relin_rescale_fused(const Context &c, int B, int ell);
void b_mul_relin_rescale(Context &c, const BatchWs &w, const MulRsItem *d_items, const u64 *relin_key, int B, int ell, hipStream_t s,
                         const Handoff &h = Handoff{});
void b_rescale(Context &c, const BatchWs &w, const RsItem *d_items, int B, int ell, hipStream_t s, const SumSrc *d_srcs = nullptr,
               const Handoff &h = Handoff{});
void hoist_rotate_hops(Context &c, const BatchWs &w, const KsItem *d_items, const KsItem *d_sources, int B, int U, int ell, hipStream_t s);
void hoist_rotate_sum(Context &c, const BatchWs &w, const KsItem *d_items, const KsItem *d_sources, int B, int U, const KsItem *d_groups, int G,
                      int ell, hipStream_t s);
bool chain_fusion_supported();
void hyb_rotate_hops(Context &c, const BatchWs &w, const KsItem *d_items, int B, int ell, hipStream_t s, int unique = 0);
void hyb_rotate_sum(Context &c, const BatchWs &w, const KsItem *d_items, int B, const KsItem *d_groups, int G, int ell, hipStream_t s, int unique = 0);
bool hyb_lazy_sum_supported(const Context &c);
void hyb_rotate_hop_single(Context &c, const Workspace &w, CtView dst, CtView src, u32 galois_elt, const u64 *galois_key, int ell, hipStream_t s);
void hyb_mul_relin(Context &c, const BatchWs &w, const MulItem *d_items, const u64 *relin_key, int B, int ell, hipStream_t s);
void hyb_keyswitch(Context &c, const Workspace &w, CtView out, const u64 *base0, const u64 *base1, const u64 *target, const u64 *key, int ell,
                   hipStream_t s);
inline int64_t ks_ntt_count(const Context &c, int ell)
{
    return c.hybrid() ? (int64_t)c.hyb_groups(ell) * (ell + c.ksp) + 2 * c.ksp + 2 * ell : (int64_t)(ell + 1) * (ell + 2);
}
void b_ew(Context &c, EwOp op, const EwItem *d_items, int B, int polys, int b_polys, int ell, hipStream_t s);
void b_add_plain(Context &c, const EwItem *d_items, int B, int ell, hipStream_t s);
void b_sum(Context &c, const SumItem *d_items, const SumSrc *d_srcs, int B, int ell, hipStream_t s);
void b_sum_group(Context &c, const SumGroup *d_groups, const SumGroupSrc *d_gsrcs, int G, int ell, hipStream_t s);
void modraise(Context &c, u64 *scratch, const EwItem *h_items, int B, int target, hipStream_t s, const EwItem *d_items = nullptr);

void f_irows_strided(const Context &c, const u64 *base, long stride, int prime_base, int period, u64 *out, long out_stride, int count,
                     hipStream_t s);
void f_irows_rot_c1(const Context &c, const KsItem *items, int ell, u64 *out, int B, hipStream_t s);
void f_irows_rs_last(const Context &c, const RsItem *items, const SumSrc *srcs, int l, u64 *out, int B, hipStream_t s);
void f_irows_rs_single(const Context &c, CtView src, int l, u64 *out, hipStream_t s);
void f_irows_decrypt(const Context &c, CtView ct, const u64 *sk, int ell, u64 *out, hipStream_t s);
void f_irows_tensor_c2(const Context &c, const MulItem *items, int ell, u64 *out, int B, hipStream_t s);
void f_irows_decrypt_items(const Context &c, const BootItem *items, const SumSrc *srcs, const u64 *sk, int ell, u64 *out, int B,
                           hipStream_t s);
void f_irows_tensor_c2_rs(const Context &c, const MulRsItem *items, int ell, u64 *out, int B, hipStream_t s);
void f_ks_frows_mac_rs(const Context &c, const u64 *ext, const MulRsItem *items, const u64 *relin_key, u64 *acc, int B, int ell, hipStream_t s);
void f_dr2_icols_lift_fcols(const Context &c, const u64 *acc, const MulRsItem *items, u64 *tmp, int B, int ell, hipStream_t s);
void f_frows_fold_final(const Context &c, const u64 *tmp, const MulRsItem *items, const u64 *acc, int B, int ell, hipStream_t s,
                        const Handoff &h = Handoff{});
void f_boot_reencode_fcols(const Context &c, const u64 *pt, u64 *ptx, const BootItem *items, int B, int ell, int t, CrtDev crt,
                           hipStream_t s);
void f_frows_boot_final(const Context &c, const u64 *ptx, const BootItem *items, int B, int t, hipStream_t s);
void f_ks_icols_lift_fcols(const Context &c, const u64 *digits, u64 *ext, int B, int ell, hipStream_t s);
void f_dr_icols_lift_fcols(const Context &c, const u64 *last, long last_stride, u64 *tmp, int polys, int cnt, int l, hipStream_t s);
void f_ks_frows_mac(const Context &c, int mode, const u64 *ext, const u64 *target, const KsItem *items, const u64 *shared_key, u64 *acc,
                    int B, int ell, hipStream_t s, bool fold_base = false);
void f_ks_lift_fcols(const Context &c, const u64 *digits, u64 *ext, int B, int ell, hipStream_t s);
void f_dr_lift_fcols(const Context &c, const u64 *last, long last_stride, u64 *tmp, int polys, int cnt, int l, hipStream_t s);
void f_frows_final(const Context &c, int mode, const u64 *tmp, const void *items, const u64 *acc, int polys, int cnt, int l,
                   hipStream_t s, RsItem single = RsItem{}, const u64 *plain = nullptr, const SumSrc *srcs = nullptr,
                   const Handoff &h = Handoff{}, bool base_folded = false);
void fill_const_plain(Context &c, u64 *out, const u64 *d_residues, int ell, hipStream_t s);
void rescale_fused(Context &c, const Workspace &w, CtView dst, CtView src, int ell, const u64 *plain, hipStream_t s);

}
```

### dacapo_amd/csrc/plan_exec.hip

```cpp
#include <math.h>
#include <string.h>

#include <algorithm>
#include <chrono>
#include <map>
#include <functional>
#include <queue>
#include <set>
#include <tuple>

#include "hevm_vm.hpp"

namespace dacapo {

#define ks_ntts(ell) ks_ntt_count(c, (ell))

template <class T>
static T *upload(const std::vector<T> &v)
{
    T *d = nullptr;
    DC_HIP_CHECK(vm_malloc(&d, std::max<size_t>(v.size(), 1) * sizeof(T)));
    if (!v.empty()) DC_HIP_CHECK(hipMemcpy(d, v.data(), v.size() * sizeof(T), hipMemcpyHostToDevice));
    return d;
}

void HEVM::build_plan()
{
    Context &c = *ctx;
    const size_t N = c.N;
    Plan &P = plan;
    for (u64 *b : P.handoff_bufs) (void)vm_free(b);
    P.handoff_bufs.clear();
    for (void *p : { (void *)P.d_enc_items, (void *)P.enc_arena, (void *)P.enc_scratch, (void *)P.d_enc_overflow })
        if (p) (void)vm_free(p);
    P.d_enc_items = nullptr, P.enc_arena = nullptr, P.enc_scratch = nullptr, P.d_enc_overflow = nullptr;
    P.enc_groups.clear(), P.enc_arena_bytes = P.enc_scratch_bytes = 0;
    if (P.d_cont_other) (void)vm_free(P.d_cont_other), P.d_cont_other = nullptr;
    if (P.d_mulrs) (void)vm_free(P.d_mulrs), P.d_mulrs = nullptr;
    for (void *p : { (void *)P.d_ks, (void *)P.d_mul, (void *)P.d_rs, (void *)P.d_ew, (void *)P.d_sum, (void *)P.d_sum_srcs, (void *)P.d_sumg, (void *)P.d_sumg_srcs, (void *)P.d_boot,
                     (void *)P.d_boot_rs, (void *)P.zenc, (void *)P.boot_ue, (void *)P.boot_tmp, (void *)P.boot_pt[0], (void *)P.boot_ptx[0],
                     (void *)P.boot_pt[1], (void *)P.boot_ptx[1] })
        if (p) (void)vm_free(p);
    P.d_boot = nullptr, P.d_boot_rs = nullptr, P.zenc = P.boot_ue = P.boot_tmp = nullptr;
    P.boot_pt[0] = P.boot_pt[1] = P.boot_ptx[0] = P.boot_ptx[1] = nullptr;
    P.boot_chunks.clear();
    if (P.graph_exec) (void)hipGraphExecDestroy(P.graph_exec);
    if (P.graph) (void)hipGraphDestroy(P.graph);
    P.graph_exec = nullptr, P.graph = nullptr;
    P.vals.clear(), P.pops.clear(), P.steps.clear();
    P.n_keyswitch = P.n_ntt = 0;
    P.n_hops = P.n_decomp = 0, P.n_fold = 0;
    const size_t nreg = ciphers.size();
    const int S = streams;
    std::vector<int> cur(nreg, -1);
    auto new_val = [&](int level, double scale) {
        Val v;
        v.level = level, v.scale = scale, v.root = (int)P.vals.size();
        P.vals.push_back(v);
        return (int)P.vals.size() - 1;
    };
    auto need = [&](int r, const char *what) {
        if (r < 0 || (size_t)r >= nreg || cur[(size_t)r] < 0) {
            fprintf(stderr, "[dacapo_amd] %s reads cipher register %d before anything wrote it\n", what, r);
            abort();
        }
        return cur[(size_t)r];
    };
    auto add_pop = [&](PopKind k, int level, std::vector<int> srcs, int dst) -> Pop & {
        Pop p;
        p.kind = k, p.level = level, p.srcs = std::move(srcs), p.dst = dst;
        P.vals[(size_t)dst].def_pop = (int)P.pops.size();
        P.pops.push_back(p);
        return P.pops.back();
    };
    for (size_t i = 0; i < header.arg_length; i++) {
        const int v = new_val((int)arg_level[i], pow(2.0, (double)arg_scale[i]));
        P.vals[(size_t)v].external = true;
        P.vals[(size_t)v].buf = home.at(i);
        cur[i] = v;
    }
    std::map<std::pair<int, u32>, int> hop_memo;
    std::map<int, int> memo_base;
    for (const WireOp &op : ops) {
        switch (op.opcode) {
        case 1: {
            int v = need(op.lhs, "rotate");
            const double in_scale = P.vals[(size_t)v].scale;
            bool memo_final = false;
            const std::vector<u32> hops = rotate_hops((int16_t)op.rhs);
            for (const u32 &elt : hops) {
                memo_final = false;
                if (rot_compose) {
                    const auto mb = memo_base.find(v);
                    auto it = hop_memo.find({ mb != memo_base.end() ? mb->second : v, elt });
                    if (it != hop_memo.end()) {
                        v = it->second;
                        memo_final = true;
                        continue;
                    }
                }
                const Val s = P.vals[(size_t)v];
                const int nv = new_val(s.level, in_scale);
                Pop &p = add_pop(P_ROT, s.level, { v }, nv);
                p.elt = elt, p.key = keys.galois.at(elt);
                p.rot = ks_hoist ? 2 : 1, p.target_level = ks_hoist ? -2 : 0;
                p.op = (int)(&op - ops.data()), p.direct = &elt == &hops.back();
                P.n_keyswitch++, P.n_ntt += ks_ntts(s.level);
                if (rot_compose) {
                    const auto mb = memo_base.find(v);
                    hop_memo[{ mb != memo_base.end() ? mb->second : v, elt }] = nv;
                }
                v = nv;
            }
            if (memo_final) {
                const Val s = P.vals[(size_t)v];
                const int nv = new_val(s.level, in_scale);
                P.vals[(size_t)nv].root = s.root;
                P.vals[(size_t)nv].def_pop = P.vals[(size_t)s.root].def_pop;
                P.vals[(size_t)v].uses++;
                const auto mb = memo_base.find(v);
                memo_base[nv] = mb != memo_base.end() ? mb->second : v;
                v = nv;
            }
            if (v == cur[op.lhs] && op.dst != op.lhs) {
                const Val s = P.vals[(size_t)v];
                const int nv = new_val(s.level, s.scale);
                add_pop(P_COPY, s.level, { v }, nv);
                v = nv;
            }
            cur[op.dst] = v;
            break;
        }
        case 2: {
            const int a = need(op.lhs, "negate");
// ... 206 lines not shown
        if ((dp = single_def(x, P_ADDP)) >= 0) p.rs_add = O[(size_t)dp].plain, x = O[(size_t)dp].srcs[0], O[(size_t)dp].dead = true;
        p.srcs[0] = x;
        if ((dp = single_def(x, P_SUM)) >= 0) {
            p.rs_sum = true;
            p.srcs = O[(size_t)dp].srcs, p.src_plain = O[(size_t)dp].src_plain;
            O[(size_t)dp].dead = true;
        }
    }

    for (Pop &p : O) {
        if (p.kind != P_BOOT || p.dead || !fold_rescale_into_boot) continue;
        const int x = p.srcs[0];
        const Val &sv = V[(size_t)x];
        const int dp = sv.root == x ? sv.def_pop : -1;
        if (dp < 0 || O[(size_t)dp].kind != P_RESCALE || O[(size_t)dp].dead || sv.uses != 1 || O[(size_t)dp].dst != x || sv.pinned) continue;
        Pop &r = O[(size_t)dp];
        p.srcs = r.srcs, p.src_plain = r.src_plain, p.rs_sum = r.rs_sum, p.rs_add = r.rs_add, p.rs_mul = r.rs_mul;
        p.level = r.level, p.boot_drop = r.level - 1, p.boot_src_scale = sv.scale;
        (void)crt_tables(p.level);
        P.n_ntt -= 2 * r.level;
        r.dead = true;
    }

    const bool seal_sums = !c.hybrid() && ks_lazy != 0;
    const bool taps_join = c.hybrid() ? double_hoist : ks_lazy == 2;
    if ((lazy_sums && hyb_lazy_sum_supported(c)) || seal_sums) {
        for (size_t ci = 0; ci < O.size(); ci++) {
            if (O[ci].dead) continue;
            if (!(O[ci].kind == P_SUM || ((O[ci].kind == P_RESCALE || O[ci].kind == P_BOOT) && O[ci].rs_sum))) continue;
            std::vector<size_t> terms;
            for (size_t k = 0; k < O[ci].srcs.size(); k++) {
                if (!O[ci].src_plain.empty() && O[ci].src_plain[k] >= 0 &&
                    !(taps_join && !online_encode && !host_encoder && dh_items.count(O[ci].src_plain[k]) && plains.at((size_t)O[ci].src_plain[k]).level >= O[ci].level))
                    continue;
                const int sidx = O[ci].srcs[k];
                const Val &sv = V[(size_t)sidx];
                const int dp = sv.root == sidx ? sv.def_pop : -1;
                if (dp < 0) continue;
                const Pop &r = O[(size_t)dp];
                if (seal_sums && !(r.rot == 2 && r.op >= 0 && ops[(size_t)r.op].opcode == 1)) continue;
                if (r.kind == P_ROT && !r.dead && r.direct && r.dst == sidx && sv.uses == 1 && !sv.pinned && r.level == O[ci].level) terms.push_back(k);
            }
            if (terms.size() < 2) continue;
            std::sort(terms.begin(), terms.end(), [&](size_t x, size_t y) { return V[(size_t)O[ci].srcs[x]].def_pop < V[(size_t)O[ci].srcs[y]].def_pop; });
            const size_t keep = terms.back();
            Pop grp = O[(size_t)V[(size_t)O[ci].srcs[keep]].def_pop];
            grp.kind = P_ROTSUM, grp.srcs.clear(), grp.direct = false, grp.op = -1;
            grp.rot = 0, grp.target_level = 0;
            for (size_t k : terms) {
                Pop &r = O[(size_t)V[(size_t)O[ci].srcs[k]].def_pop];
                grp.srcs.push_back(r.srcs[0]), grp.elts.push_back(r.elt), grp.keys.push_back(r.key), grp.ops.push_back(r.op);
                grp.plains.push_back(O[ci].src_plain.empty() ? -1 : O[ci].src_plain[k]);
                r.dead = true;
                if (k != keep) V[(size_t)O[ci].srcs[k]].uses = 0, V[(size_t)O[ci].srcs[k]].def_pop = -1;
            }
            const int gi = V[(size_t)O[ci].srcs[keep]].def_pop;
            O[(size_t)gi] = grp;
            std::vector<int> srcs, plain;
            for (size_t k = 0; k < O[ci].srcs.size(); k++)
                if (k == keep || std::find(terms.begin(), terms.end(), k) == terms.end()) {
                    srcs.push_back(O[ci].srcs[k]);
                    if (!O[ci].src_plain.empty()) plain.push_back(k == keep ? -1 : O[ci].src_plain[k]);
                }
            O[ci].srcs = srcs, O[ci].src_plain = plain;
            if (O[ci].kind == P_SUM && O[ci].srcs.size() == 1 && (O[ci].src_plain.empty() || O[ci].src_plain[0] < 0)) {
                const int old = O[(size_t)gi].dst, dst = O[ci].dst;
                if (V[(size_t)dst].root == dst && V[(size_t)dst].level == V[(size_t)old].level) {
                    O[(size_t)gi].dst = dst;
                    V[(size_t)dst].def_pop = gi;
                    V[(size_t)old].uses = 0, V[(size_t)old].def_pop = -1;
                    O[ci].dead = true;
                }
            }
        }
    }

    if (double_hoist) {
        std::vector<int> need_sp;
        for (const Pop &p : O)
            if (!p.dead && p.kind == P_ROTSUM)
                for (int pl : p.plains)
                    if (pl >= 0) need_sp.push_back(pl);
        ensure_special_limbs(need_sp);
    }

    int max_wave = 0;
    for (Pop &p : O) {
        if (p.dead) continue;
        int w = 0;
        for (int s : p.srcs) {
            const int dp = V[(size_t)s].def_pop;
            if (dp >= 0) w = std::max(w, O[(size_t)dp].wave);
        }
        p.wave = w + 1;
        max_wave = std::max(max_wave, p.wave);
    }

    std::vector<std::vector<int>> by_wave((size_t)max_wave + 1);
    for (size_t i = 0; i < O.size(); i++)
        if (!O[i].dead) by_wave[(size_t)O[i].wave].push_back((int)i);
    std::vector<KsItem> h_ks;
    std::vector<MulItem> h_mul;
    std::vector<MulRsItem> h_mulrs;
    std::vector<RsItem> h_rs;
    std::vector<EwItem> h_ew;
    std::vector<SumItem> h_sum;
    std::vector<SumGroup> h_sumg;
    std::vector<SumGroupSrc> h_sumg_srcs;
    double sum_stat[5] = { 0, 0, 0, 0, 0 };
    std::vector<SumSrc> h_srcs;
    std::vector<std::vector<int>> step_pops;
    std::map<int, int> fold_rs_of;
    std::vector<char> absorbed(O.size(), 0);
    std::map<size_t, std::vector<int>> fold_pops;
    if (ks_fold_rescale && !online_encode && !c.hybrid()) {
        std::map<int, bool> constant;
        auto is_constant = [&](int reg) {
            auto it = constant.find(reg);
            if (it != constant.end()) return it->second;
            const Plain &pl = plains.at((size_t)reg);
            bool same = pl.d != nullptr;
            if (same) {
                std::vector<u64> h((size_t)pl.level * N);
                DC_HIP_CHECK(hipMemcpy(h.data(), pl.d, h.size() * sizeof(u64), hipMemcpyDeviceToHost));
                for (size_t i = 0; i < (size_t)pl.level && same; i++)
                    for (size_t k = 1; k < N && same; k++) same = h[i * N + k] == h[i * N];
            }
            return constant[reg] = same;
        };
        for (size_t ri = 0; ri < O.size(); ri++) {
            const Pop &rp = O[ri];
            if (rp.dead || rp.kind != P_RESCALE || rp.rs_sum || rp.srcs.size() != 1) continue;
            const Val &mv = V[(size_t)rp.srcs[0]];
            if (mv.root != rp.srcs[0] || mv.def_pop < 0 || mv.uses != 1 || mv.pinned) continue;
            Pop &mp = O[(size_t)mv.def_pop];
            if (mp.dead || mp.kind != P_MULCC || mp.dst != rp.srcs[0] || mp.level != rp.level || mp.level < 2) continue;
            if (rp.rs_mul >= 0 && !is_constant(rp.rs_mul)) continue;
            fold_rs_of[mv.def_pop] = (int)ri, mp.target_level = -3;
        }
    }
    for (int w = 1; w <= max_wave; w++) {
        std::map<std::tuple<int, int, int>, std::vector<int>> buckets;
        for (int pi : by_wave[(size_t)w])
            if (!absorbed[(size_t)pi])
                buckets[std::make_tuple((int)O[(size_t)pi].kind, O[(size_t)pi].level, O[(size_t)pi].target_level)].push_back(pi);
        for (auto &kv : buckets) {
            const PopKind kind = (PopKind)std::get<0>(kv.first);
            if (kind == P_ROT && std::get<2>(kv.first) == -2)
                std::stable_sort(kv.second.begin(), kv.second.end(), [&](int x, int y) {
                    const Pop &a = O[(size_t)x], &b = O[(size_t)y];
                    return a.srcs[0] != b.srcs[0] ? a.srcs[0] < b.srcs[0] : a.elt < b.elt;
                });
            else if (kind == P_ROT && !c.hybrid() && option(OPT_KS_ITEMS_FAST))
                std::stable_sort(kv.second.begin(), kv.second.end(), [&](int x, int y) { return O[(size_t)x].elt < O[(size_t)y].elt; });
            const bool heavy = kind == P_ROT || kind == P_MULCC || kind == P_RESCALE || kind == P_BOOT || kind == P_ROTSUM;
            const size_t chunk = std::max<size_t>(1, (heavy ? (size_t)max_batch : (size_t)4096) / (size_t)S);
            if (kind == P_ROTSUM) {
                for (size_t off = 0; off < kv.second.size();) {
                    size_t end = off, items = 0;
                    while (end < kv.second.size() && (items == 0 || items + O[(size_t)kv.second[end]].srcs.size() <= chunk))
                        items += O[(size_t)kv.second[end]].srcs.size(), end++;
                    Step st;
                    st.kind = kind, st.level = std::get<1>(kv.first), st.wave = w, st.count = (int)items;
                    std::vector<int> members(kv.second.begin() + (long)off, kv.second.begin() + (long)end);
                    for (int pi : members) O[(size_t)pi].step = (int)P.steps.size();
                    P.steps.push_back(st);
// ... 184 lines not shown
        DC_HIP_CHECK(vm_malloc(&P.d_enc_overflow, sizeof(int)));
        DC_HIP_CHECK(hipMemset(P.d_enc_overflow, 0, sizeof(int)));
        P.d_enc_items = upload(h_items);
        size_t gi = 0;
        for (auto &kv : groups)
            for (size_t k0 = 0; k0 < kv.second.size(); k0 += (size_t)chunk, gi++) {
                Plan::EncGroup &g = P.enc_groups[gi];
                g.out = P.enc_arena + placed[gi].first;
                for (int k = 0; k < g.count; k++) plains.at((size_t)kv.second[k0 + (size_t)k]).d = g.out + (size_t)k * (size_t)g.level * N;
            }
        for (auto &kv : online.items)
            if (!use.count(kv.first)) plains.at((size_t)kv.first).d = P.enc_arena;
    }
    for (const Pop &p : O) {
        if (p.dead) continue;
        V[(size_t)V[(size_t)p.dst].root].def_step = p.step;
        for (int s : p.srcs) {
            Val &r = V[(size_t)V[(size_t)s].root];
            r.last_use = std::max(r.last_use, p.step);
        }
    }
    const size_t buf_elems = (size_t)2 * c.K * N;
    std::vector<u64 *> free_list = P.pool;
    typedef std::pair<int, u64 *> Rel;
    std::priority_queue<Rel, std::vector<Rel>, std::greater<Rel>> busy;
    size_t live = 0;
    P.max_live = 0;
    std::vector<std::vector<int>> defs(P.steps.size());
    for (size_t v = 0; v < V.size(); v++)
        if (V[v].root == (int)v && V[v].def_step >= 0 && !V[v].external) defs[(size_t)V[v].def_step].push_back((int)v);
    for (size_t s = 0; s < P.steps.size(); s++) {
        while (!busy.empty() && P.steps[(size_t)busy.top().first].wave < P.steps[s].wave) {
            free_list.push_back(busy.top().second);
            busy.pop();
            live--;
        }
        for (int v : defs[s]) {
            u64 *b;
            if (!free_list.empty()) {
                b = free_list.back();
                free_list.pop_back();
            } else {
                DC_HIP_CHECK(vm_malloc(&b, buf_elems * (size_t)S * sizeof(u64)));
                P.pool.push_back(b);
            }
            V[(size_t)v].buf = b;
            live++;
            P.max_live = std::max(P.max_live, live);
            if (!V[(size_t)v].pinned) busy.push({ std::max(V[(size_t)v].last_use, (int)s), b });
        }
    }
    const long ps = (long)c.K * (long)N;
    auto view = [&](int v, int sidx) {
        u64 *b = V[(size_t)V[(size_t)v].root].buf;
        if (!b) {
            fprintf(stderr, "[dacapo_amd] plan: value %d has no buffer (internal error)\n", v);
            abort();
        }
        return CtView{ b + (size_t)sidx * buf_elems, ps };
    };
    size_t need_t = 0, need_d = 0, need_e = 0, need_a = 0, need_m = 0;
    size_t need_bpt = 0, need_bptx = 0;
    int boot_tmax = 0;
    std::vector<std::pair<int, int>> h_boot_pops;
    std::vector<double> h_boot_ratio;
    P.launches = 0;
    for (size_t s = 0; s < P.steps.size(); s++) {
        Step &st = P.steps[s];
        st.count *= S;
        const size_t B = (size_t)st.count, l = (size_t)st.level;
        switch (st.kind) {
        case P_ROT:
            st.first = (int)h_ks.size();
            {
                const bool hoisted = st.target == -2;
                std::map<const u64 *, u32> slot_of;
                std::vector<KsItem> sources;
                for (int pi : step_pops[s])
                    for (int q = 0; q < S; q++) {
                        const CtView sv = view(O[(size_t)pi].srcs[0], q);
                        if (hoisted && !slot_of.count(sv.p)) sources.push_back(KsItem{ sv, sv, nullptr, 1u, 0 });
                        const u32 slot = (c.hybrid() || hoisted) ? slot_of.emplace(sv.p, (u32)slot_of.size()).first->second : 0u;
                        h_ks.push_back(KsItem{ sv, view(O[(size_t)pi].dst, q), O[(size_t)pi].key, O[(size_t)pi].elt, slot });
                    }
                st.unique = (int)slot_of.size();
                st.gfirst = (int)h_ks.size(), st.gcount = (int)sources.size();
                h_ks.insert(h_ks.end(), sources.begin(), sources.end());
                for (int pi : step_pops[s])
                    if (O[(size_t)pi].rot) P.n_hops += S, P.n_decomp += hoisted ? 0 : S;
                if (hoisted) P.n_decomp += st.unique;
            }
            break;
        case P_ROTSUM: {
            st.first = (int)h_ks.size();
            std::map<const u64 *, u32> slot_of;
            std::vector<KsItem> groups, sources;
            for (int pi : step_pops[s])
                for (int q = 0; q < S; q++) {
                    const Pop &rp = O[(size_t)pi];
                    const CtView dst = view(rp.dst, q);
                    groups.push_back(KsItem{ dst, dst, nullptr, (u32)(h_ks.size() - (size_t)st.first), (u32)rp.srcs.size() });
                    std::vector<size_t> order(rp.srcs.size());
                    for (size_t k = 0; k < order.size(); k++) order[k] = k;
                    if (!c.hybrid()) std::stable_sort(order.begin(), order.end(), [&](size_t x, size_t y) { return rp.srcs[x] < rp.srcs[y]; });
                    for (size_t k : order) {
                        const CtView sv = view(rp.srcs[k], q);
                        if (!c.hybrid() && !slot_of.count(sv.p)) sources.push_back(KsItem{ sv, sv, nullptr, 1u, 0 });
                        const u32 slot = slot_of.emplace(sv.p, (u32)slot_of.size()).first->second;
                        const int pl = rp.plains.empty() ? -1 : rp.plains[k];
                        h_ks.push_back(KsItem{ sv, dst, rp.keys[k], rp.elts[k], slot, pl >= 0 ? plains.at((size_t)pl).d : nullptr,
                                               pl >= 0 ? plains.at((size_t)pl).dsp : nullptr });
                    }
                }
            st.unique = (int)slot_of.size();
            P.n_hops += (int64_t)(h_ks.size() - (size_t)st.first);
            P.n_decomp += c.hybrid() ? (int64_t)(h_ks.size() - (size_t)st.first) : (int64_t)st.unique;
            st.gfirst = (int)h_ks.size(), st.gcount = (int)groups.size();
            h_ks.insert(h_ks.end(), groups.begin(), groups.end());
            h_ks.insert(h_ks.end(), sources.begin(), sources.end());
            break;
        }
        case P_MULCC:
            if (st.fold_rs) {
                st.first = (int)h_mulrs.size();
                const std::vector<int> &rs = fold_pops.at(s);
                for (size_t k = 0; k < rs.size(); k++)
                    for (int q = 0; q < S; q++) {
                        const Pop &mp = O[(size_t)step_pops[s][k]], &rp = O[(size_t)rs[k]];
                        MulRsItem it;
                        it.a = view(mp.srcs[0], q), it.b = view(mp.srcs[1], q), it.dst = view(rp.dst, q);
                        if (rp.rs_add >= 0) it.add = plains.at((size_t)rp.rs_add).d;
                        if (rp.rs_mul >= 0) it.mul = plains.at((size_t)rp.rs_mul).d, it.mul_stride = (long)N;
                        h_mulrs.push_back(it);
                    }
                P.n_fold += (int64_t)B;
                break;
            }
            st.first = (int)h_mul.size();
            for (int pi : step_pops[s])
                for (int q = 0; q < S; q++)
                    h_mul.push_back(MulItem{ view(O[(size_t)pi].srcs[0], q), view(O[(size_t)pi].srcs[1], q), view(O[(size_t)pi].dst, q) });
            break;
        case P_RESCALE:
            st.first = (int)h_rs.size();
            for (int pi : step_pops[s])
                for (int q = 0; q < S; q++) {
                    const Pop &rp = O[(size_t)pi];
                    RsItem it{ view(rp.srcs[0], q), view(rp.dst, q), 0, 0, nullptr, nullptr };
                    if (rp.rs_sum) {
                        it.first = (int)h_srcs.size(), it.count = (int)rp.srcs.size();
                        for (size_t k = 0; k < rp.srcs.size(); k++) {
                            const int pl = rp.src_plain.empty() ? -1 : rp.src_plain[k];
                            h_srcs.push_back(SumSrc{ view(rp.srcs[k], q), pl >= 0 ? plains.at((size_t)pl).d : nullptr });
                        }
                    }
                    if (rp.rs_add >= 0) it.add = plains.at((size_t)rp.rs_add).d;
                    if (rp.rs_mul >= 0) it.mul = plains.at((size_t)rp.rs_mul).d;
                    h_rs.push_back(it);
                }
            break;
        case P_SUM:
            st.first = (int)h_sum.size();
            if (option(OPT_TRACE)) {
                std::map<std::vector<int>, int> lists;
                std::set<int> distinct;
                size_t terms = 0;
// ... 228 lines not shown
        for (size_t ai = 0; ai < P.steps.size(); ai++)
            if (P.steps[ai].fused_consumer >= 0 && P.steps[ai].h.cont == CONT_MUL) P.steps[ai].h.other = P.d_cont_other + other_first[ai];
    }
    auto alloc = [&](size_t limbs) {
        u64 *d = nullptr;
        DC_HIP_CHECK(vm_malloc(&d, std::max<size_t>(limbs, 1) * N * sizeof(u64)));
        return d;
    };
    for (int ln = 0; ln < 2; ln++) {
        BatchWs &w = P.ws[ln];
        for (void *p : { (void *)w.target, (void *)w.digits, (void *)w.ext, (void *)w.acc, (void *)w.tmp })
            if (p) (void)vm_free(p);
        w = BatchWs{};
        if (ln >= plan_lanes) continue;
        w.target = alloc(need_t), w.digits = alloc(need_d), w.ext = alloc(need_e);
        w.acc = alloc(need_a), w.tmp = alloc(need_m);
    }
    {
        size_t aux_waves = 0;
        for (size_t i = 0; i < P.steps.size(); i++)
            if (P.steps[i].lane == 1 && (i == 0 || P.steps[i - 1].wave != P.steps[i].wave || P.steps[i - 1].lane != 1)) aux_waves++;
        while (P.events.size() < 2 * aux_waves + 2) {
            hipEvent_t e;
            DC_HIP_CHECK(hipEventCreateWithFlags(&e, hipEventDisableTiming));
            P.events.push_back(e);
        }
        if (aux_waves && !aux_stream) DC_HIP_CHECK(hipStreamCreateWithFlags(&aux_stream, hipStreamNonBlocking));
    }
    P.n_keyswitch *= S, P.n_ntt *= S;
    P.ready = true;
    if (plan_graph) capture_plan();
    if (option(OPT_TRACE)) {
        static const char *kn[] = { "rot", "mulcc", "rescale", "sum", "neg", "mulp", "addp", "copy", "boot", "modraise", "rotsum" };
        size_t nsteps[kPopKinds] = { 0 }, nitems[kPopKinds] = { 0 };
        std::map<std::pair<int, int>, std::pair<size_t, size_t>> ks;
        for (const Step &st : P.steps) {
            nsteps[st.kind]++, nitems[st.kind] += (size_t)st.count;
            if (st.kind == P_ROT || st.kind == P_MULCC || st.kind == P_RESCALE || st.kind == P_BOOT || st.kind == P_ROTSUM) {
                auto &e = ks[{ (int)st.kind, st.level }];
                e.first++, e.second += (size_t)st.count;
            }
        }
        if (option(OPT_TRACE) >= 2) {
            int lastw = -1;
            for (size_t i = 0; i < P.steps.size() && i < 400; i++) {
                const Step &st = P.steps[i];
                if (st.wave != lastw) fprintf(stderr, "\n  wave %d:", st.wave);
                fprintf(stderr, " [%s l%d x%d%s]", kn[st.kind], st.level, st.count, st.lane ? " aux" : "");
                lastw = st.wave;
            }
            fprintf(stderr, "\n");
        }
        for (int k = 0; k < kPopKinds; k++)
            if (nsteps[k]) fprintf(stderr, "[dacapo_amd] plan:   %-8s %5zu steps %6zu items\n", kn[k], nsteps[k], nitems[k]);
        {
            size_t gsteps = 0, ggroups = 0, gitems = 0;
            for (const Step &st : P.steps)
                if (st.kind == P_SUM && st.gcount > 0) gsteps++, ggroups += (size_t)st.gcount, gitems += (size_t)st.count;
            fprintf(stderr, "[dacapo_amd] plan:   sums sharing sources: %zu steps run %zu items as %zu groups\n", gsteps, gitems, ggroups);
        }
        fprintf(stderr, "[dacapo_amd] plan:   sums, in limbs: %.0f terms (each 2 ciphertext limbs + at most 1 plaintext limb read), %.0f items (2 limbs written); "
                        "distinct sources per step %.0f; ciphertext reads with equal source lists 4 / 8 to a thread %.0f / %.0f\n",
                sum_stat[0], sum_stat[3], sum_stat[1], sum_stat[2], sum_stat[4]);
        {
            std::map<std::tuple<int, int, int, int>, int> edges;
            std::vector<std::vector<int>> users(V.size());
            for (size_t i = 0; i < O.size(); i++)
                if (!O[i].dead)
                    for (int sv : O[i].srcs) users[(size_t)sv].push_back((int)i);
            for (size_t i = 0; i < O.size(); i++) {
                if (O[i].dead) continue;
                const int d = O[i].dst;
                const int nu = (int)users[(size_t)d].size() + (V[(size_t)d].pinned ? 100 : 0);
                if (users[(size_t)d].empty()) edges[std::make_tuple((int)O[i].kind, -1, nu, 0)]++;
                for (int u : users[(size_t)d]) edges[std::make_tuple((int)O[i].kind, (int)O[(size_t)u].kind, nu, O[(size_t)u].wave - O[i].wave)]++;
            }
            for (auto &kv : edges)
                fprintf(stderr, "[dacapo_amd] plan edge: %-8s -> %-8s uses %3d wave distance %3d : %d\n", kn[std::get<0>(kv.first)],
                        std::get<1>(kv.first) < 0 ? "(none)" : kn[std::get<1>(kv.first)], std::get<2>(kv.first), std::get<3>(kv.first), kv.second);
        }
        for (auto &kv : ks)
            fprintf(stderr, "[dacapo_amd] plan:   %-8s level %2d: %5zu steps %6zu items\n", kn[kv.first.first], kv.first.second,
                    kv.second.first, kv.second.second);
    }
    if (option(OPT_TRACE))
        fprintf(stderr, "[dacapo_amd] plan: %zu ops -> %zu pseudo-ops -> %zu steps (%zu on the auxiliary stream, %zu fused into their producer's last kernel) in %d waves, ~%zu launches, %zu live buffers (%.1f GB pool)\n",
                ops.size(), O.size(), P.steps.size(), (size_t)std::count_if(P.steps.begin(), P.steps.end(), [](const Step &st) { return st.lane == 1; }), P.n_fused,
                max_wave, P.launches, P.max_live, (double)P.pool.size() * buf_elems * 8 / 1e9);
}

void HEVM::issue_step(const Step &st, hipStream_t q)
{
    Context &c = *ctx;
    Plan &P = plan;
    const BatchWs &w = P.ws[st.lane];
    switch (st.kind) {
    case P_ROT:
        if (st.target == -2) {
            hoist_rotate_hops(c, w, P.d_ks + st.first, P.d_ks + st.gfirst, st.count, st.unique, st.level, q);
            break;
        }
        b_rotate_hops(st.target < 0 ? *bctx : c, w, P.d_ks + st.first, st.count, st.level, q, st.h, st.unique); break;
    case P_ROTSUM:
        if (!c.hybrid()) {
            hoist_rotate_sum(c, w, P.d_ks + st.first, P.d_ks + st.gfirst + st.gcount, st.count, st.unique, P.d_ks + st.gfirst, st.gcount, st.level, q);
            break;
        }
        hyb_rotate_sum(c, w, P.d_ks + st.first, st.count, P.d_ks + st.gfirst, st.gcount, st.level, q, st.unique); break;
    case P_MULCC:
        if (st.fold_rs) {
            b_mul_relin_rescale(c, w, P.d_mulrs + st.first, keys.relin, st.count, st.level, q, st.h);
            break;
        }
        b_mul_relin(c, w, P.d_mul + st.first, keys.relin, st.count, st.level, q, st.h); break;
    case P_RESCALE: b_rescale(c, w, P.d_rs + st.first, st.count, st.level, q, P.d_sum_srcs, st.h); break;
    case P_SUM:
        if (st.gcount > 0)
            b_sum_group(c, P.d_sumg + st.gfirst, P.d_sumg_srcs, st.gcount, st.level, q);
        else
            b_sum(c, P.d_sum + st.first, P.d_sum_srcs, st.count, st.level, q);
        break;
    case P_NEG: b_ew(c, EwOp::Neg, P.d_ew + st.first, st.count, 2, 2, st.level, q); break;
    case P_COPY: b_ew(c, EwOp::Copy, P.d_ew + st.first, st.count, 2, 2, st.level, q); break;
    case P_MODRAISE: modraise(c, w.digits, P.h_ew.data() + st.first, st.count, st.target, q, P.d_ew + st.first); break;
    case P_MULP: b_ew(c, EwOp::Mul, P.d_ew + st.first, st.count, 2, 1, st.level, q); break;
    case P_ADDP: b_add_plain(c, P.d_ew + st.first, st.count, st.level, q); break;
    case P_BOOT: plan_boot_step(st.first, st.count, st.level, st.target, st.lane, q, st.h); break;
    }
}

void HEVM::issue_plan(hipStream_t s)
{
    Context &c = *ctx;
    Plan &P = plan;
    if (test_zero_enc) {
        if (P.zenc) DC_HIP_CHECK(hipMemsetAsync(P.zenc, 0, P.zenc_bytes, s));
    } else
        for (const Plan::BootChunk &bc : P.boot_chunks) plan_zero_encrypt(bc.first, bc.count, bc.target, s);
    const bool step_profile = option(OPT_STEP_PROFILE) != 0 && !plan_graph;
    std::map<std::tuple<int, int, int>, std::pair<int, double>> prof;
    double wave_max = 0, wave_sum = 0, crit_path = 0, all_steps = 0;
    size_t waves_seen = 0, wide_waves = 0;
    size_t ev = 0, eg = 0;
    for (size_t a = 0; a < P.steps.size();) {
        size_t b = a;
        bool has_aux = false;
        while (b < P.steps.size() && P.steps[b].wave == P.steps[a].wave) has_aux |= P.steps[b].lane == 1, b++;
        for (; eg < P.enc_groups.size() && P.enc_groups[eg].wave <= P.steps[a].wave; eg++) {
            const Plan::EncGroup &g = P.enc_groups[eg];
            enc_batch(c, enc_tables, online.d_consts, P.d_enc_items + g.first, g.count, g.level, P.enc_scratch, g.out, P.d_enc_overflow, s);
        }
        if (has_aux) {
            DC_HIP_CHECK(hipEventRecord(P.events[ev], s));
            DC_HIP_CHECK(hipStreamWaitEvent(aux_stream, P.events[ev], 0));
            ev++;
        }
        for (size_t i = a; i < b; i++) {
            const Step &st = P.steps[i];
            hipStream_t q = st.lane ? aux_stream : s;
            issue_step(st, q);
            if (step_profile) {
                static auto t_prev = std::chrono::steady_clock::now();
                if (i == 0) {
                    DC_HIP_CHECK(hipStreamSynchronize(s));
                    t_prev = std::chrono::steady_clock::now();
                }
                DC_HIP_CHECK(hipStreamSynchronize(q));
                const auto t1 = std::chrono::steady_clock::now();
                const int bucket = st.count <= 1 ? 1 : st.count <= 2 ? 2 : st.count <= 4 ? 4 : st.count <= 8 ? 8 : st.count <= 32 ? 32 : 128;
                auto &e = prof[std::make_tuple((int)st.kind, st.level, bucket)];
                const double dt = std::chrono::duration<double>(t1 - t_prev).count();
                e.first++, e.second += dt;
                wave_max = std::max(wave_max, dt), wave_sum += dt;
                t_prev = t1;
            }
        }
        if (has_aux) {
            DC_HIP_CHECK(hipEventRecord(P.events[ev], aux_stream));
            DC_HIP_CHECK(hipStreamWaitEvent(s, P.events[ev], 0));
            ev++;
        }
        if (step_profile) {
            crit_path += wave_max, all_steps += wave_sum, waves_seen++, wide_waves += (b - a) > 1;
            wave_max = wave_sum = 0;
        }
// ... 71 lines not shown
            if (ty == hipGraphNodeTypeKernel) {
                hipKernelNodeParams kp;
                DC_HIP_CHECK(hipGraphKernelNodeGetParams(cur, &kp));
                DC_HIP_CHECK(hipGraphAddKernelNode(&nw, main, dp, nd, &kp));
            } else if (ty == hipGraphNodeTypeMemset) {
                hipMemsetParams mp;
                DC_HIP_CHECK(hipGraphMemsetNodeGetParams(cur, &mp));
                DC_HIP_CHECK(hipGraphAddMemsetNode(&nw, main, dp, nd, &mp));
            } else
                ok = false;
            tail = nw;
            auto it = next.find(cur);
            cur = it == next.end() ? nullptr : it->second;
        }
        (void)hipGraphDestroy(g);
        return tail;
    };
    hipGraphNode_t zenc_tail = add_unit([&](hipStream_t s) {
        if (test_zero_enc) {
            if (P.zenc) DC_HIP_CHECK(hipMemsetAsync(P.zenc, 0, P.zenc_bytes, s));
        } else
            for (const Plan::BootChunk &bc : P.boot_chunks) plan_zero_encrypt(bc.first, bc.count, bc.target, s);
    }, {});
    struct Ref { int lane = -1; long seq = -1; hipGraphNode_t node = nullptr; };
    std::map<const u64 *, Ref> writer;
    std::map<const u64 *, Ref> reader[2];
    Ref lane_tail[2] = { Ref{ 0, 0, zenc_tail }, Ref{ 1, 0, zenc_tail } };
    long seq = 0;
    for (size_t i = 0; i < P.steps.size() && ok; i++) {
        const Step &st = P.steps[i];
        const int other = 1 - st.lane;
        Ref cross;
        auto need = [&](const Ref &r) {
            if (r.node && r.lane == other && r.seq > cross.seq) cross = r;
        };
        for (const u64 *b : st.reads) {
            auto it = writer.find(b);
            if (it != writer.end()) need(it->second);
        }
        for (const u64 *b : st.writes) {
            auto it = writer.find(b);
            if (it != writer.end()) need(it->second);
            auto rt = reader[other].find(b);
            if (rt != reader[other].end()) need(rt->second);
        }
        std::vector<hipGraphNode_t> deps{ lane_tail[st.lane].node };
        if (cross.node) deps.push_back(cross.node);
        const hipGraphNode_t tail = add_unit([&](hipStream_t s) { issue_step(st, s); }, deps);
        if (!tail) continue;
        const Ref me{ st.lane, ++seq, tail };
        lane_tail[st.lane] = me;
        for (const u64 *b : st.reads) reader[st.lane][b] = me;
        for (const u64 *b : st.writes) writer[b] = me;
    }
    if (ok) (void)add_unit([&](hipStream_t s) { bump_epoch(s); }, { lane_tail[0].node, lane_tail[1].node });
    if (!ok) {
        (void)hipGraphDestroy(main);
        return false;
    }
    P.graph = main;
    DC_HIP_CHECK(hipGraphInstantiate(&P.graph_exec, P.graph, nullptr, nullptr, 0));
    return true;
}

void HEVM::drop_plan_graph()
{
    Plan &P = plan;
    if (P.graph_exec) (void)hipGraphExecDestroy(P.graph_exec);
    if (P.graph) (void)hipGraphDestroy(P.graph);
    P.graph_exec = nullptr, P.graph = nullptr;
}

void HEVM::run_plan()
{
    if (!plan.ready) build_plan();
    Context &c = *ctx;
    Plan &P = plan;
    cur = 0;
    hipStream_t s = S();
    memset(op_counts, 0, sizeof(op_counts));
    for (const WireOp &op : ops)
        if (op.opcode <= 10) op_counts[op.opcode]++;
    n_keyswitch = P.n_keyswitch, n_ntt = P.n_ntt;
    n_hops = P.n_hops, n_decomp = P.n_decomp, n_fold = P.n_fold;
    t_bootstrap = 0.0;
    const long ps = (long)c.K * (long)c.N;
    if (plan_graph) {
        capture_plan();
        if (P.graph_exec)
            DC_HIP_CHECK(hipGraphLaunch(P.graph_exec, s));
        else
            issue_plan(s);
    } else
        issue_plan(s);
    DC_HIP_CHECK(hipStreamSynchronize(s));
    if (P.d_enc_overflow) {
        int overflow = 0;
        DC_HIP_CHECK(hipMemcpy(&overflow, P.d_enc_overflow, sizeof(int), hipMemcpyDeviceToHost));
        if (overflow) {
            fprintf(stderr, "[dacapo_amd] encode: coefficient does not fit 120 bits (scale too large)\n");
            abort();
        }
    }
    for (size_t r = 0; r < P.final_val.size() && r < ciphers.size(); r++) {
        const int v = P.final_val[r];
        if (v < 0) continue;
        reg_base[r] = P.vals[(size_t)P.vals[(size_t)v].root].buf;
        ciphers[r].data = reg_base[r] + (size_t)sel * (size_t)2 * c.K * c.N;
        ciphers[r].poly_stride = ps;
        ciphers[r].level = P.vals[(size_t)v].level;
        ciphers[r].scale = P.vals[(size_t)v].scale;
    }
}

}
```

### dacapo_amd/lowlevel.py

```python
from __future__ import annotations

import ctypes as C

import numpy as np

from . import LIB_PATH, LIB_PATH_GW

_lib = None
_libs: dict = {}


def lib_gw():
    return lib(LIB_PATH_GW)


def lib(path=None):
    global _lib
    if path is not None and str(path) != str(LIB_PATH):
        if str(path) not in _libs:
            _libs[str(path)] = _bind(path)
        return _libs[str(path)]
    if _lib is None:
        _lib = _bind(LIB_PATH)
    return _lib


def loaded_libs():
    return ([_lib] if _lib is not None else []) + list(_libs.values())


def _bind(path):
    if True:
        if not path.exists():
            raise RuntimeError(f"{path} is missing: run `python -c 'import __graft_entry__ as g; g.build()'` "
                               "(there is no CPU fallback for the HEVM hot path)")
        L = C.CDLL(str(path))
        vp, u64p, i32, lng = C.c_void_p, C.c_void_p, C.c_int, C.c_long
        L.dc_context_create.restype = vp
        L.dc_context_create.argtypes = [i32, i32, i32, vp]
        L.dc_context_create_hybrid.restype = vp
        L.dc_context_create_hybrid.argtypes = [i32, i32, i32, i32]
        L.dc_context_create_hybrid_primes.restype = vp
        L.dc_context_create_hybrid_primes.argtypes = [i32, vp, i32, i32, i32]
        L.dc_context_key_digits.argtypes = [vp]
        L.dc_context_max_level.argtypes = [vp]
        L.dc_context_destroy.argtypes = [vp]
        L.dc_context_logn.argtypes = [vp]
        L.dc_context_num_primes.argtypes = [vp]
        L.dc_context_primes.argtypes = [vp, vp]
        L.dc_context_roots.argtypes = [vp, vp]
        L.dc_malloc.restype = vp
        L.dc_malloc.argtypes = [C.c_size_t]
        L.dc_free.argtypes = [vp]
        L.dc_memcpy_h2d.argtypes = [vp, vp, C.c_size_t]
        L.dc_memcpy_d2h.argtypes = [vp, vp, C.c_size_t]
        L.dc_memset.argtypes = [vp, i32, C.c_size_t]
        L.dc_memcpy_d2d.argtypes = [vp, vp, C.c_size_t, vp]
        L.dc_stream_sync.argtypes = [vp]
        L.dc_set_device.argtypes = [i32]
        L.dc_event_create.restype = vp
        L.dc_event_destroy.argtypes = [vp]
        L.dc_event_record.argtypes = [vp, vp]
        L.dc_event_elapsed_ms.restype = C.c_float
        L.dc_event_elapsed_ms.argtypes = [vp, vp]
        for f in (L.dc_ntt_forward, L.dc_ntt_inverse):
            f.argtypes = [vp, u64p, lng, i32, vp, i32, i32, vp]
        L.dc_ntt_variant.argtypes = [vp, i32, i32, u64p, lng, i32, vp, i32, i32, vp]
        L.dc_ct_negate.argtypes = [vp, u64p, lng, u64p, lng, i32, vp]
        L.dc_ct_add.argtypes = [vp, u64p, lng, u64p, lng, u64p, lng, i32, vp]
        L.dc_ct_add_plain.argtypes = [vp, u64p, lng, u64p, lng, u64p, i32, vp]
        L.dc_ct_mul_plain.argtypes = [vp, u64p, lng, u64p, lng, u64p, i32, vp]
        L.dc_ct_mul_relin.argtypes = [vp, u64p, lng, u64p, lng, u64p, lng, u64p, i32, vp]
        L.dc_ct_mul_relin_rescale.argtypes = [vp, u64p, lng, u64p, lng, u64p, lng, u64p, u64p, vp, i32, vp]
        L.dc_ct_rotate_hop.argtypes = [vp, u64p, lng, u64p, lng, C.c_uint32, u64p, i32, vp]
        L.dc_ct_rotate_hoisted.argtypes = [vp, vp, lng, u64p, lng, vp, vp, i32, i32, vp]
        L.dc_ct_rotate_sum_hoisted.argtypes = [vp, u64p, lng, vp, lng, vp, vp, vp, vp, i32, i32, vp]
        L.dc_ct_rescale.argtypes = [vp, u64p, lng, u64p, lng, i32, vp]
        L.dc_ct_modswitch.argtypes = [vp, u64p, lng, u64p, lng, i32, i32, vp]
        L.dc_keyswitch.argtypes = [vp, u64p, lng, u64p, u64p, u64p, u64p, i32, vp]
        L.dc_galois_ntt.argtypes = [vp, u64p, lng, u64p, lng, C.c_uint32, i32, i32, vp]
        L.dc_poly_mul.argtypes = [vp, u64p, u64p, u64p, i32, vp]
        L.dc_poly_add.argtypes = [vp, u64p, u64p, u64p, i32, vp]
        L.dc_galois_elt_from_step.restype = C.c_uint32
        L.dc_galois_elt_from_step.argtypes = [vp, i32]
        from .runner import bind_options

        bind_options(L)
    return L


class DeviceBuffer:

    def __init__(self, shape, dtype=np.uint64):
        self.shape = tuple(int(x) for x in np.atleast_1d(shape))
        self.dtype = np.dtype(dtype)
        self.nbytes = int(np.prod(self.shape)) * self.dtype.itemsize
        self.ptr = lib().dc_malloc(max(self.nbytes, 16))

    @classmethod
    def from_host(cls, a: np.ndarray):
        a = np.ascontiguousarray(a)
        d = cls(a.shape, a.dtype)
        lib().dc_memcpy_h2d(d.ptr, a.ctypes.data, a.nbytes)
        return d

    def to_host(self) -> np.ndarray:
        out = np.empty(self.shape, dtype=self.dtype)
        lib().dc_memcpy_d2h(out.ctypes.data, self.ptr, self.nbytes)
        return out

    def at(self, elem_offset: int) -> int:
        return self.ptr + int(elem_offset) * self.dtype.itemsize

    def __del__(self):
        try:
            if self.ptr:
                lib().dc_free(self.ptr)
                self.ptr = None
        except Exception:
            pass


def read_device(ptr: int, shape, dtype=np.uint64) -> np.ndarray:
    out = np.empty(shape, dtype=dtype)
    lib().dc_memcpy_d2h(out.ctypes.data, ptr, out.nbytes)
    return out


class Context:
    def __init__(self, logN=15, num_primes=14, bit_size=60, primes=None, special=1, alpha=None):
        narrow = bit_size != 60 or (primes is not None and any(int(p).bit_length() != 60 for p in primes))
        L = lib_gw() if narrow else lib()
        self.L = L
        arr = None
        if primes is not None:
            arr = (C.c_uint64 * len(primes))(*[int(p) for p in primes])
            num_primes = len(primes)
        alpha = special if alpha is None else alpha
        if (special, alpha) != (1, 1) and primes is not None:
            self.h = L.dc_context_create_hybrid_primes(logN, arr, num_primes, special, alpha)
        elif (special, alpha) != (1, 1):
            assert bit_size == 60
            self.h = L.dc_context_create_hybrid(logN, num_primes, special, alpha)
        else:
            self.h = L.dc_context_create(logN, num_primes, bit_size, arr)
        self.key_digits, self.max_level = int(L.dc_context_key_digits(self.h)), int(L.dc_context_max_level(self.h))
        self.logN, self.N, self.K = logN, 1 << logN, num_primes
        out = np.zeros(num_primes, dtype=np.uint64)
        L.dc_context_primes(self.h, out.ctypes.data)
        self.primes = [int(x) for x in out]
        L.dc_context_roots(self.h, out.ctypes.data)
        self.roots = [int(x) for x in out]

    def __del__(self):
        try:
            self.L.dc_context_destroy(self.h)
        except Exception:
# ... 17 lines not shown
```

### dacapo_amd/runner.py

```python
from __future__ import annotations

import contextlib
import ctypes
import re
import weakref
from pathlib import Path

import numpy as np

from . import LIB_PATH

lw = None


def reinit_lw():
    global lw
    if lw is None:
        lw = bind_vm_lib(LIB_PATH)
    return lw


_vm_libs: dict = {}


def bind_vm_lib(path):
    if str(path) in _vm_libs:
        return _vm_libs[str(path)]
    if not Path(path).exists():
        raise RuntimeError(f"{path} is missing: build it with __graft_entry__.build() (no CPU fallback exists)")
    L = _vm_libs[str(path)] = ctypes.CDLL(str(path))
    L.initFullVM.argtypes = [ctypes.c_char_p, ctypes.c_bool]
    L.initFullVM.restype = ctypes.c_void_p
    L.initClientVM.argtypes = [ctypes.c_char_p]
    L.initClientVM.restype = ctypes.c_void_p
    L.initServerVM.argtypes = [ctypes.c_char_p]
    L.initServerVM.restype = ctypes.c_void_p
    L.create_context.argtypes = [ctypes.c_char_p]
    L.load.argtypes = [ctypes.c_void_p, ctypes.c_char_p, ctypes.c_char_p]
    L.loadClient.argtypes = [ctypes.c_void_p, ctypes.c_void_p]
    L.getArgLen.argtypes = [ctypes.c_void_p]
    L.getArgLen.restype = ctypes.c_int64
    L.getResLen.argtypes = [ctypes.c_void_p]
    L.getResLen.restype = ctypes.c_int64
    L.encrypt.argtypes = [ctypes.c_void_p, ctypes.c_int64, ctypes.POINTER(ctypes.c_double), ctypes.c_int]
    L.decrypt.argtypes = [ctypes.c_void_p, ctypes.c_int64, ctypes.POINTER(ctypes.c_double)]
    L.decrypt_result.argtypes = [ctypes.c_void_p, ctypes.c_int64, ctypes.POINTER(ctypes.c_double)]
    L.getResIdx.argtypes = [ctypes.c_void_p, ctypes.c_int64]
    L.getResIdx.restype = ctypes.c_int64
    L.getCtxt.argtypes = [ctypes.c_void_p, ctypes.c_int64]
    L.getCtxt.restype = ctypes.c_void_p
    L.preprocess.argtypes = [ctypes.c_void_p]
    L.run.argtypes = [ctypes.c_void_p]
    L.setDebug.argtypes = [ctypes.c_void_p, ctypes.c_bool]
    L.setToGPU.argtypes = [ctypes.c_void_p, ctypes.c_bool]
    L.printMem.argtypes = [ctypes.c_void_p]
    L.hevm_init_fresh.argtypes = [ctypes.c_int, ctypes.c_int]
    L.hevm_init_fresh.restype = ctypes.c_void_p
    L.hevm_init_fresh_primes.argtypes = [ctypes.c_int, ctypes.POINTER(ctypes.c_uint64), ctypes.c_int]
    L.hevm_init_fresh_primes.restype = ctypes.c_void_p
    L.has_test_hooks = hasattr(L, "hevm_init_seeded")
    if L.has_test_hooks:
        L.hevm_init_seeded.argtypes = [ctypes.c_int, ctypes.c_int, ctypes.c_uint64]
        L.hevm_init_seeded.restype = ctypes.c_void_p
        L.hevm_init_seeded_primes.argtypes = [ctypes.c_int, ctypes.POINTER(ctypes.c_uint64), ctypes.c_int, ctypes.c_uint64]
        L.hevm_init_seeded_primes.restype = ctypes.c_void_p
        L.hevm_secret_key.argtypes = [ctypes.c_void_p]
        L.hevm_secret_key.restype = ctypes.c_void_p
        L.hevm_test_zero_encryption.argtypes = [ctypes.c_void_p, ctypes.c_bool]
    L.hevm_context.argtypes = [ctypes.c_void_p]
    L.hevm_context.restype = ctypes.c_void_p
    for f in (L.hevm_relin_key, L.hevm_public_key):
        f.argtypes = [ctypes.c_void_p]
        f.restype = ctypes.c_void_p
    L.hevm_key_buffers.argtypes = [ctypes.c_void_p, ctypes.c_void_p, ctypes.c_void_p, ctypes.c_int]
    L.hevm_key_digest.argtypes = [ctypes.c_void_p]
    L.hevm_key_digest.restype = ctypes.c_uint64
    L.hevm_keys_replaced.argtypes = [ctypes.c_void_p]
    L.hevm_boot_switch_keys.argtypes = [ctypes.c_void_p, ctypes.POINTER(ctypes.c_void_p), ctypes.POINTER(ctypes.c_void_p),
                                        ctypes.POINTER(ctypes.c_int)]
    L.hevm_boot_switch_keys.restype = ctypes.c_int
    L.hevm_galois_key.argtypes = [ctypes.c_void_p, ctypes.c_uint32]
    L.hevm_galois_key.restype = ctypes.c_void_p
    L.hevm_plain.argtypes = [ctypes.c_void_p, ctypes.c_int64, ctypes.POINTER(ctypes.c_int32), ctypes.POINTER(ctypes.c_double)]
    L.hevm_plain.restype = ctypes.c_void_p
    L.hevm_plain_special.argtypes = [ctypes.c_void_p, ctypes.c_int64]
    L.hevm_plain_special.restype = ctypes.c_void_p
    L.hevm_load_mem.argtypes = [ctypes.c_void_p, ctypes.c_char_p, ctypes.c_uint64, ctypes.c_char_p, ctypes.c_uint64]
    L.hevm_last_run_stats.argtypes = [ctypes.c_void_p, ctypes.POINTER(ctypes.c_int64), ctypes.POINTER(ctypes.c_int64),
                                       ctypes.POINTER(ctypes.c_int64)]
    L.hevm_last_run_hoist_stats.argtypes = [ctypes.c_void_p, ctypes.POINTER(ctypes.c_int64), ctypes.POINTER(ctypes.c_int64)]
    L.hevm_last_run_fold_rescale_stats.argtypes = [ctypes.c_void_p, ctypes.POINTER(ctypes.c_int64)]
    L.hevm_plan_lazy_groups.argtypes = [ctypes.c_void_p, ctypes.POINTER(ctypes.c_int32), ctypes.c_int64]
    L.hevm_plan_lazy_groups.restype = ctypes.c_int64
    L.hevm_set_streams.argtypes = [ctypes.c_void_p, ctypes.c_int]
    L.hevm_select_stream.argtypes = [ctypes.c_void_p, ctypes.c_int]
    L.hevm_last_run_bootstrap_seconds.argtypes = [ctypes.c_void_p]
    L.hevm_last_run_bootstrap_seconds.restype = ctypes.c_double
    L.hevm_plaintext_bytes.argtypes = [ctypes.c_void_p]
    L.hevm_plaintext_bytes.restype = ctypes.c_uint64
    L.hevm_destroy.argtypes = [ctypes.c_void_p]
    L.hevm_destroy.restype = None
    L.hevm_add_rotation_keys.argtypes = [ctypes.c_void_p, ctypes.POINTER(ctypes.c_int64), ctypes.c_int]
    L.hevm_save_ctxt.argtypes = [ctypes.c_void_p, ctypes.c_int64, ctypes.c_char_p]
    L.hevm_load_ctxt.argtypes = [ctypes.c_void_p, ctypes.c_int64, ctypes.c_char_p]
    bind_options(L)
    for name, value in _cli_options.items():
        L.hevm_set_option(name.encode(), int(value))
    return L


_cli_options: dict = {}


def bind_options(L):
    L.hevm_set_option.argtypes = [ctypes.c_char_p, ctypes.c_longlong]
    L.hevm_get_option.argtypes = [ctypes.c_char_p]
    L.hevm_get_option.restype = ctypes.c_longlong
    L.hevm_reset_options.argtypes = []
    return L


def _option_libs():
    from . import lowlevel

    reinit_lw()
    libs, seen = [], set()
    for L in list(_vm_libs.values()) + lowlevel.loaded_libs():
        if L._name not in seen:
            seen.add(L._name)
            libs.append(L)
    return libs


def set_option(name: str, value: int):
    for L in _option_libs():
        L.hevm_set_option(name.encode(), int(value))


def get_option(name: str) -> int:
    reinit_lw()
    return int(lw.hevm_get_option(name.encode()))


def apply_cli_options(argv):
    out, i = [], 0
    while i < len(argv):
        if argv[i] == "--opt" and i + 1 < len(argv):
            name, _, value = argv[i + 1].partition("=")
            set_option(name, int(value, 0))
            _cli_options[name] = int(value, 0)
            i += 2
        else:
            out.append(argv[i])
            i += 1
    return out


@contextlib.contextmanager
def options(**kw):
    libs = _option_libs()
    for L in libs:
        bind_options(L)
    old = [{k: int(L.hevm_get_option(k.encode())) for k in kw} for L in libs]
    try:
        for k, v in kw.items():
            set_option(k, v)
        yield
    finally:
        for L, saved in zip(libs, old):
            for k, v in saved.items():
                L.hevm_set_option(k.encode(), v)


class hevm_ctxt(ctypes.Structure):
    _fields_ = [("data", ctypes.c_void_p), ("poly_stride", ctypes.c_int64), ("level", ctypes.c_int32),
# ... 106 lines not shown
        self.lw.printMem(self.vm)

    def setInput(self, i, data):
        if not isinstance(data, np.ndarray):
            data = np.array(data, dtype=np.float64)
        data = np.ascontiguousarray(data, dtype=np.float64)
        carr = data.ctypes.data_as(ctypes.POINTER(ctypes.c_double))
        self.lw.encrypt(self.vm, i, carr, len(data))

    def setDebug(self, enable):
        self.lw.setDebug(self.vm, enable)

    def setToGPU(self, ongpu):
        self.lw.setToGPU(self.vm, ongpu)

    def getOutput(self):
        result = np.zeros((self.reslen, self.slots), dtype=np.float64)
        data = np.zeros(self.slots, dtype=np.float64)
        for i in range(self.reslen):
            carr = data.ctypes.data_as(ctypes.POINTER(ctypes.c_double))
            self.lw.decrypt_result(self.vm, i, carr)
            result[i] = data
        return result

    def keyBuffers(self):
        n = self.lw.hevm_key_buffers(self.vm, None, None, 0)
        ptrs, words = (ctypes.c_void_p * n)(), (ctypes.c_uint64 * n)()
        self.lw.hevm_key_buffers(self.vm, ptrs, words, n)
        return [(int(ptrs[i] or 0), int(words[i])) for i in range(n)]

    def keyDigest(self) -> int:
        return int(self.lw.hevm_key_digest(self.vm))

    def keysReplaced(self):
        self.lw.hevm_keys_replaced(self.vm)

    def close(self):
        if getattr(self, "vm", None) and self.vm in _live_vms:
            self.lw.hevm_destroy(self.vm)
            _live_vms.pop(self.vm, None)
        self.vm = None

    def plaintextBytes(self) -> int:
        return int(self.lw.hevm_plaintext_bytes(self.vm))

    def addRotationKeys(self, offsets):
        arr = (ctypes.c_int64 * len(offsets))(*[int(o) for o in offsets])
        self.lw.hevm_add_rotation_keys(self.vm, arr, len(offsets))

    def saveCtxt(self, reg: int, path):
        self.lw.hevm_save_ctxt(self.vm, reg, str(path).encode("utf-8"))

    def loadCtxt(self, reg: int, path):
        self.lw.hevm_load_ctxt(self.vm, reg, str(path).encode("utf-8"))

    def getResIdx(self, i: int) -> int:
        return int(self.lw.getResIdx(self.vm, i))

    def getCtxt(self, reg: int) -> hevm_ctxt:
        return hevm_ctxt.from_address(self.lw.getCtxt(self.vm, reg))

    def lazy_groups(self):
        n = self.lw.hevm_plan_lazy_groups(self.vm, None, 0)
        if n <= 0:
            return []
        buf = (ctypes.c_int32 * n)()
        self.lw.hevm_plan_lazy_groups(self.vm, buf, n)
        out, i = [], 0
        while i < n:
            out.append(list(buf[i + 1 : i + 1 + buf[i]]))
            i += 1 + buf[i]
        return out

    def hoist_stats(self):
        hops, dec = ctypes.c_int64(), ctypes.c_int64()
        self.lw.hevm_last_run_hoist_stats(self.vm, ctypes.byref(hops), ctypes.byref(dec))
        return {"hops": hops.value, "decompositions": dec.value}

    def fold_rescale_stats(self):
        pairs = ctypes.c_int64()
        self.lw.hevm_last_run_fold_rescale_stats(self.vm, ctypes.byref(pairs))
        return pairs.value

    def stats(self):
        counts = (ctypes.c_int64 * 11)()
        ks, ntt = ctypes.c_int64(), ctypes.c_int64()
        self.lw.hevm_last_run_stats(self.vm, counts, ctypes.byref(ks), ctypes.byref(ntt))
        return {"op_counts": list(counts), "keyswitches": ks.value, "ntts": ntt.value,
                "bootstrap_s": float(self.lw.hevm_last_run_bootstrap_seconds(self.vm))}

    def printer(self, latency, rms, mem_usage=0.0):
        bench = re.search(r"optimized/(.*)/(.*)\.(.*)\._", self.hevm_path)
        print("======================================")
        print("---------------Option-----------------")
        if bench:
            print("compiler:", bench.group(1))
            print("benchname:", bench.group(2))
            print("waterline:", bench.group(3))
        print("library:", run_library)
        print("device:", run_hardware)
        print("---------------Result-----------------")
        print("latency:", latency)
        print("rms:", rms)
        print("======================================")
        print()
```

### include/dacapo_ckks.h

```cpp
#ifndef DACAPO_CKKS_H
#define DACAPO_CKKS_H

#include <stddef.h>
#include <stdint.h>

#ifdef __cplusplus
extern "C" {
#endif
#if defined(__GNUC__)
#pragma GCC visibility push(default)
#endif

typedef struct dc_context dc_context;

dc_context *dc_context_create(int logN, int num_primes, int bit_size, const uint64_t *primes);
dc_context *dc_context_create_hybrid(int logN, int num_primes, int special, int alpha);
dc_context *dc_context_create_hybrid_primes(int logN, const uint64_t *primes, int num_primes, int special, int alpha);
int dc_context_key_digits(const dc_context *ctx);
int dc_context_max_level(const dc_context *ctx);
void dc_context_destroy(dc_context *ctx);
int dc_context_logn(const dc_context *ctx);
int dc_context_num_primes(const dc_context *ctx);
void dc_context_primes(const dc_context *ctx, uint64_t *out );
void dc_context_roots(const dc_context *ctx, uint64_t *out );

void *dc_malloc(size_t bytes);
void dc_free(void *dptr);
void dc_memcpy_h2d(void *dst, const void *src, size_t bytes);
void dc_memcpy_d2h(void *dst, const void *src, size_t bytes);
void dc_memset(void *dst, int value, size_t bytes);
void dc_memcpy_d2d(void *dst, const void *src, size_t bytes, void *stream);
void dc_stream_sync(void *stream);
void dc_set_device(int device);
void dc_device_sync(void);
int dc_device_count(void);
void dc_mem_info(uint64_t *free_bytes, uint64_t *total_bytes);
void *dc_event_create(void);
void dc_event_destroy(void *event);
void dc_event_record(void *event, void *stream);
float dc_event_elapsed_ms(void *start, void *stop);

void dc_ntt_forward(dc_context *ctx, uint64_t *data, long limb_stride, int count, const int32_t *d_prime_idx, int prime_base,
                    int prime_period, void *stream);
void dc_ntt_inverse(dc_context *ctx, uint64_t *data, long limb_stride, int count, const int32_t *d_prime_idx, int prime_base,
                    int prime_period, void *stream);

void dc_ntt_variant(dc_context *ctx, int variant, int inverse, uint64_t *data, long limb_stride, int count, const int32_t *d_prime_idx,
                    int prime_base, int prime_period, void *stream);

void dc_ct_negate(dc_context *ctx, uint64_t *dst, long dst_stride, const uint64_t *a, long a_stride, int ell, void *stream);
void dc_ct_add(dc_context *ctx, uint64_t *dst, long dst_stride, const uint64_t *a, long a_stride, const uint64_t *b,
               long b_stride, int ell, void *stream);
void dc_ct_add_plain(dc_context *ctx, uint64_t *dst, long dst_stride, const uint64_t *a, long a_stride, const uint64_t *plain,
                     int ell, void *stream);
void dc_ct_mul_plain(dc_context *ctx, uint64_t *dst, long dst_stride, const uint64_t *a, long a_stride, const uint64_t *plain,
                     int ell, void *stream);
void dc_ct_mul_relin(dc_context *ctx, uint64_t *dst, long dst_stride, const uint64_t *a, long a_stride, const uint64_t *b,
                     long b_stride, const uint64_t *relin_key, int ell, void *stream);
void dc_ct_mul_relin_rescale(dc_context *ctx, uint64_t *dst, long dst_stride, const uint64_t *a, long a_stride, const uint64_t *b,
                             long b_stride, const uint64_t *relin_key, const uint64_t *add_plain, const uint64_t *mul_const, int ell,
                             void *stream);
void dc_ct_rotate_hop(dc_context *ctx, uint64_t *dst, long dst_stride, const uint64_t *src, long src_stride,
                      uint32_t galois_elt, const uint64_t *galois_key, int ell, void *stream);
void dc_ct_rotate_hoisted(dc_context *ctx, uint64_t *const *dsts, long dst_stride, const uint64_t *src, long src_stride,
                          const uint32_t *galois_elts, const uint64_t *const *galois_keys, int count, int ell, void *stream);
void dc_ct_rotate_sum_hoisted(dc_context *ctx, uint64_t *dst, long dst_stride, const uint64_t *const *srcs, long src_stride,
                              const uint32_t *galois_elts, const uint64_t *const *galois_keys, const uint64_t *const *plains,
                              const uint64_t *const *plains_sp, int count, int ell, void *stream);
void dc_ct_rescale(dc_context *ctx, uint64_t *dst, long dst_stride, const uint64_t *src, long src_stride, int ell,
                   void *stream);
void dc_ct_modswitch(dc_context *ctx, uint64_t *dst, long dst_stride, const uint64_t *src, long src_stride, int ell, int down,
                     void *stream);

void dc_keyswitch(dc_context *ctx, uint64_t *out, long out_stride, const uint64_t *base0, const uint64_t *base1,
                  const uint64_t *target, const uint64_t *key, int ell, void *stream);
void dc_galois_ntt(dc_context *ctx, uint64_t *dst, long dst_stride, const uint64_t *src, long src_stride, uint32_t galois_elt,
                   int polys, int ell, void *stream);
void dc_poly_mul(dc_context *ctx, uint64_t *dst, const uint64_t *a, const uint64_t *b, int ell, void *stream);
void dc_poly_add(dc_context *ctx, uint64_t *dst, const uint64_t *a, const uint64_t *b, int ell, void *stream);

uint32_t dc_galois_elt_from_step(const dc_context *ctx, int step);

#if defined(__GNUC__)
#pragma GCC visibility pop
#endif
#ifdef __cplusplus
}
#endif
#endif
```

### include/hevm_abi.h

```cpp
#ifndef HEVM_ABI_H
#define HEVM_ABI_H

#include <stdbool.h>
#include <stdint.h>

#ifdef __cplusplus
extern "C" {
#endif
#if defined(__GNUC__)
#pragma GCC visibility push(default)
#endif

void *initFullVM(char *dir, bool device);
void *initClientVM(char *dir);
void *initServerVM(char *dir);
void create_context(char *dir);
void load(void *vm, char *constant, char *vmfile);
void loadClient(void *vm, void *is);
void encrypt(void *vm, int64_t i, double *dat, int len);
void decrypt(void *vm, int64_t i, double *dat);
void decrypt_result(void *vm, int64_t i, double *dat);
int64_t getResIdx(void *vm, int64_t i);
void *getCtxt(void *vm, int64_t id);
void preprocess(void *vm);
void run(void *vm);
int64_t getArgLen(void *vm);
int64_t getResLen(void *vm);
void setDebug(void *vm, bool enable);
void setToGPU(void *vm, bool ongpu);
void printMem(void *vm);

struct hevm_ctxt {
    uint64_t *data;
    int64_t poly_stride;
    int32_t level;
    int32_t reserved;
    double scale;
};

void *hevm_init_fresh(int logN, int num_primes);
void *hevm_init_fresh_primes(int logN, const uint64_t *primes, int num_primes);
#ifdef DC_TEST_HOOKS
void *hevm_init_seeded(int logN, int num_primes, uint64_t seed);
void *hevm_init_seeded_primes(int logN, const uint64_t *primes, int num_primes, uint64_t seed);
const uint64_t *hevm_secret_key(void *vm);
void hevm_test_zero_encryption(void *vm, bool on);
#endif
void *hevm_context(void *vm);
const uint64_t *hevm_relin_key(void *vm);
const uint64_t *hevm_galois_key(void *vm, uint32_t elt);
const uint64_t *hevm_public_key(void *vm);
int hevm_boot_switch_keys(void *vm, const uint64_t **down, const uint64_t **up, int *down_limbs);
int hevm_key_buffers(void *vm, uint64_t **ptrs, uint64_t *words, int cap);
uint64_t hevm_key_digest(void *vm);
void hevm_keys_replaced(void *vm);
const uint64_t *hevm_plain(void *vm, int64_t i, int32_t *level, double *scale);
const uint64_t *hevm_plain_special(void *vm, int64_t i);
void hevm_load_mem(void *vm, const void *cst, uint64_t cst_len, const void *hevm, uint64_t hevm_len);
void hevm_last_run_stats(void *vm, int64_t *op_counts , int64_t *keyswitches, int64_t *ntts);
void hevm_last_run_hoist_stats(void *vm, int64_t *hops, int64_t *decompositions);
void hevm_last_run_fold_rescale_stats(void *vm, int64_t *pairs);
int64_t hevm_plan_lazy_groups(void *vm, int32_t *out, int64_t cap);
void hevm_set_streams(void *vm, int n);
void hevm_select_stream(void *vm, int s);
double hevm_last_run_bootstrap_seconds(void *vm);
uint64_t hevm_plaintext_bytes(void *vm);
void hevm_destroy(void *vm);
void hevm_add_rotation_keys(void *vm, const int64_t *offsets, int count);
void hevm_save_ctxt(void *vm, int64_t reg, const char *path);
void hevm_load_ctxt(void *vm, int64_t reg, const char *path);

int hevm_set_option(const char *name, long long value);
long long hevm_get_option(const char *name);
void hevm_reset_options(void);

void hevm_seal_parms_id(uint64_t poly_modulus_degree, const uint64_t *primes, int count, uint64_t out[4]);
void hevm_seal_save_parms(const char *path, int compr_mode, uint64_t poly_modulus_degree, const uint64_t *primes, int count);
int hevm_seal_load_parms(const char *path, uint64_t *poly_modulus_degree, uint64_t *primes, int capacity);
void hevm_seal_save_ciphertext(const char *path, int compr_mode, uint64_t poly_modulus_degree, const uint64_t *primes, int limbs, int size,
                               int is_ntt, double scale, const uint64_t *data);
int64_t hevm_seal_load_ciphertext(const char *path, uint64_t *poly_modulus_degree, int *limbs, int *size, int *is_ntt, double *scale,
                                  uint64_t parms_id[4], uint64_t *data, uint64_t capacity);
int hevm_seal_zstd_available(void);
void hevm_chacha20_block(const uint32_t key[8], uint64_t counter, uint64_t nonce, uint32_t out[16]);
void hevm_chacha20_blocks_device(const uint32_t key[8], uint64_t counter, uint64_t nonce, int blocks, uint32_t *out_host);

#if defined(__GNUC__)
#pragma GCC visibility pop
#endif
#ifdef __cplusplus
}
#endif
#endif
```

Baseline: 1.323 million NTT/s.

## Fold two-term ciphertext sums into the producing rotation's final kernel

```diff
diff --git a/dacapo_amd/csrc/batch_ops.hip b/dacapo_amd/csrc/batch_ops.hip
--- a/dacapo_amd/csrc/batch_ops.hip
+++ b/dacapo_amd/csrc/batch_ops.hip
@@ -95,7 +95,7 @@
 
 template <int MODE>
 static void b_ks_tail(Context &c, const BatchWs &w, u64 *digits, const KsItem *items, const void *final_items, const u64 *shared_key, int B,
-                      int ell, hipStream_t s, const Handoff &h)
+                      int ell, hipStream_t s, const Handoff &h, bool with_add = false)
 {
     const size_t N = c.N;
     const int K = c.K, sp = K - 1;
@@ -121,18 +121,33 @@
         f_dr_lift_fcols(c, acc_last, acc_ps, w.tmp, 2 * B, ell, sp, s);
     } else
         f_dr_icols_lift_fcols(c, acc_last, acc_ps, w.tmp, 2 * B, ell, sp, s);
-    f_frows_final(c, (MODE == 1 && fused_mac) ? 4 : MODE, w.tmp, final_items, w.acc, 2 * B, ell, sp, s, RsItem{}, nullptr, nullptr, h,
+    f_frows_final(c, (MODE == 1 && fused_mac) ? 4 : (MODE == 0 && with_add) ? 5 : MODE, w.tmp, final_items, w.acc, 2 * B, ell, sp, s, RsItem{}, nullptr, nullptr, h,
                   MODE == 0 && fused_mac);
 }
 
-void b_rotate_hops(Context &c, const BatchWs &w, const KsItem *d_items, int B, int ell, hipStream_t s, const Handoff &h, int unique)
+__global__ __launch_bounds__(kBT) void b_ks_add_kernel(const KsItem *__restrict__ items, size_t N, const DModulus *__restrict__ mods)
+{
+    const int i = blockIdx.y, p = blockIdx.z & 1, b = blockIdx.z >> 1;
+    const KsItem it = items[b];
+    if (!it.add.p) return;
+    const u64 q = mods[i].q;
+    const size_t k = ((size_t)blockIdx.x * kBT + threadIdx.x) * 2;
+    u64x2 *o = reinterpret_cast<u64x2 *>(it.dst.limb(p, i, N) + k);
+    const u64x2 a = *o, w = *reinterpret_cast<const u64x2 *>(it.add.limb(p, i, N) + k);
+    *o = u64x2{ addmod(a.x, w.x, q), addmod(a.y, w.y, q) };
+}
+
+void b_rotate_hops(Context &c, const BatchWs &w, const KsItem *d_items, int B, int ell, hipStream_t s, const Handoff &h, int unique, bool with_add)
 {
     if (c.hybrid()) {
         hyb_rotate_hops(c, w, d_items, B, ell, s, unique);
         return;
     }
+    const bool split = with_add && h.cont == CONT_NONE && (long)B * ell >= (long)option(OPT_ROT_ADD_SPLIT_LIMBS);
     f_irows_rot_c1(c, d_items, ell, w.digits, B, s);
-    b_ks_tail<0>(c, w, w.digits, d_items, d_items, nullptr, B, ell, s, h);
+    b_ks_tail<0>(c, w, w.digits, d_items, d_items, nullptr, B, ell, s, h, with_add && !split);
+    if (split)
+        DC_LAUNCH(b_ks_add_kernel, dim3((unsigned)(c.N / (2 * kBT)), (unsigned)ell, (unsigned)(2 * B)), dim3(kBT), 0, s, d_items, c.N, c.d_mods);
 }
 
 void b_mul_relin(Context &c, const BatchWs &w, const MulItem *d_items, const u64 *relin_key, int B, int ell, hipStream_t s, const Handoff &h)
diff --git a/dacapo_amd/csrc/c_api.hip b/dacapo_amd/csrc/c_api.hip
--- a/dacapo_amd/csrc/c_api.hip
+++ b/dacapo_amd/csrc/c_api.hip
@@ -288,6 +288,24 @@
     const KsItem it{ V(src, src_stride), V(dst, dst_stride), galois_key, galois_elt, 0 };
     const KsItem *d = static_cast<const KsItem *>(item_slot(ctx, &it, sizeof(it), S(stream)));
     b_rotate_hops(*ctx->c, batch_ws(ctx->c->ws0), d, 1, ell, S(stream));
+}
+void dc_ct_rotate_hop_add(dc_context *ctx, uint64_t *dst, long dst_stride, const uint64_t *src, long src_stride, const uint64_t *add,
+                          long add_stride, uint32_t galois_elt, const uint64_t *galois_key, int ell, void *stream)
+{
+    Context &c = *ctx->c;
+    if (c.hybrid()) {
+        fprintf(stderr, "[dacapo_amd] dc_ct_rotate_hop_add: this context switches keys with grouped digits; the call is for SEAL-layout keys\n");
+        abort();
+    }
+    if (!add || overlaps(dst, src) || overlaps(dst, add) || ell < 1 || ell > c.max_level()) {
+        fprintf(stderr, "[dacapo_amd] dc_ct_rotate_hop_add: dst must alias neither src nor add, add must be given, level 1..%d (got %d)\n",
+                c.max_level(), ell);
+        abort();
+    }
+    KsItem it{ V(src, src_stride), V(dst, dst_stride), galois_key, galois_elt, 0 };
+    it.add = V(add, add_stride);
+    const KsItem *d = static_cast<const KsItem *>(item_slot(ctx, &it, sizeof(it), S(stream)));
+    b_rotate_hops(c, batch_ws(c.ws0), d, 1, ell, S(stream), Handoff{}, 0, true);
 }
 void dc_ct_rotate_hoisted(dc_context *ctx, uint64_t *const *dsts, long dst_stride, const uint64_t *src, long src_stride,
                           const uint32_t *galois_elts, const uint64_t *const *galois_keys, int count, int ell, void *stream)
diff --git a/dacapo_amd/csrc/fused_ks.hip b/dacapo_amd/csrc/fused_ks.hip
--- a/dacapo_amd/csrc/fused_ks.hip
+++ b/dacapo_amd/csrc/fused_ks.hip
@@ -358,11 +358,13 @@
     const DModulus M = mods[i];
     const u64 inv = inv_last[(size_t)l * Kp + i];
     const u64 *in = tmp + (size_t)z * N;
-    if (MODE == 0 && base_folded) {
+    constexpr bool ROT = MODE == 0 || MODE == 5, ADD = MODE == 5;
+    if (ROT && base_folded) {
         constexpr int E = 1 << LOGE;
         const KsItem it = reinterpret_cast<const KsItem *>(items_)[b];
         const u64 *x = acc + (((size_t)bp) * (cnt + 1) + i) * N;
         u64 *o = it.dst.limb(p, i, N);
+        const u64 *ad = (ADD && it.add.p) ? it.add.limb(p, i, N) : nullptr;
         u64 v[E];
         auto nost = [](int, u64) {};
         ntt_tile_x<K, LOGE, false, false, true, false, true>(v, M, tw + ((size_t)i << logN), logN, blockIdx.x, [=](int gi) { return in[gi]; }, nost, lds);
@@ -372,18 +374,24 @@
             const u64x2 a = *reinterpret_cast<const u64x2 *>(x + g0 + j);
             u64x2 r;
             r.x = mulmod(submod(a.x, v[j], M.q), inv, M), r.y = mulmod(submod(a.y, v[j + 1], M.q), inv, M);
+            if (ADD && ad) {
+                const u64x2 w = *reinterpret_cast<const u64x2 *>(ad + g0 + j);
+                r.x = addmod(r.x, w.x, M.q), r.y = addmod(r.y, w.y, M.q);
+            }
             *reinterpret_cast<u64x2 *>(o + g0 + j) = r;
         }
-    } else if (MODE == 0) {
+    } else if (ROT) {
         const KsItem it = reinterpret_cast<const KsItem *>(items_)[b];
         const u64 *x = acc + (((size_t)bp) * (cnt + 1) + i) * N;
         const u64 *c0 = it.src.limb(0, i, N);
         u64 *o = it.dst.limb(p, i, N);
+        const u64 *ad = (ADD && it.add.p) ? it.add.limb(p, i, N) : nullptr;
         ntt_tile<K, LOGE, false, false, true>(
             M, tw + ((size_t)i << logN), logN, blockIdx.x, [=](int g) { return in[g]; },
             [=](int g, u64 v) {
                 const u64 base = p == 0 ? c0[galois_idx((u32)g, it.elt, logN)] : 0;
-                o[g] = addmod(base, mulmod(submod(x[g], v, M.q), inv, M), M.q);
+                const u64 r = addmod(base, mulmod(submod(x[g], v, M.q), inv, M), M.q);
+                o[g] = (ADD && ad) ? addmod(r, ad[g], M.q) : r;
             },
             lds);
     } else if (MODE == 1) {
@@ -480,15 +488,17 @@
             v[j] = addmod(base, mulmod(submod(ac[g[j]], x[j], M.q), inv, M), M.q);
             o[g[j]] = v[j];
         }
-    } else if (MODE == 0) {
+    } else if (MODE == 0 || MODE == 5) {
         const KsItem it = reinterpret_cast<const KsItem *>(items_)[b];
         const u64 *ac = acc + (((size_t)(b * 2 + p)) * (cnt + 1) + i) * N;
         const u64 *c0 = it.src.limb(0, i, N);
         u64 *o = it.dst.limb(p, i, N);
+        const u64 *ad = (MODE == 5 && it.add.p) ? it.add.limb(p, i, N) : nullptr;
 #pragma unroll
         for (int j = 0; j < E; j++) {
             const u64 base = (p == 0 && !base_folded) ? c0[galois_idx((u32)g[j], it.elt, logN)] : 0;
             v[j] = addmod(base, mulmod(submod(ac[g[j]], x[j], M.q), inv, M), M.q);
+            if (MODE == 5 && ad) v[j] = addmod(v[j], ad[g[j]], M.q);
             o[g[j]] = v[j];
         }
     } else {
@@ -1082,6 +1092,8 @@
             DC_CONT(2, CONT_BOOT);
         } else if (mode == 0 && h.cont == CONT_BOOT) {
             DC_CONT(0, CONT_BOOT);
+        } else if (mode == 5 && h.cont == CONT_BOOT) {
+            DC_CONT(5, CONT_BOOT);
         } else {
             fprintf(stderr, "[dacapo_amd] f_frows_final: no continuation kernel for mode %d -> consumer kind %d\n", mode, h.cont);
             abort();
@@ -1097,6 +1109,7 @@
     case 1: DC_FINAL(1); break;
     case 2: DC_FINAL(2); break;
     case 4: DC_FINAL(4); break;
+    case 5: DC_FINAL(5); break;
     default: DC_FINAL(3); break;
     }
 #undef DC_FINAL
diff --git a/dacapo_amd/csrc/hevm_vm.hip b/dacapo_amd/csrc/hevm_vm.hip
--- a/dacapo_amd/csrc/hevm_vm.hip
+++ b/dacapo_amd/csrc/hevm_vm.hip
@@ -418,6 +418,7 @@
                         "is an approximate base conversion, and dividing by P q in one exact pass does not reproduce it\n", ksp, alpha);
         abort();
     }
+    rot_add_fold = option(OPT_ROT_ADD_FOLD) != 0;
     const int bits = (int)option(OPT_PRIME_BITS);
     ctx.reset(new Context(logN, K, bits, primes, ksp, alpha));
     ctx->ensure_scratch();
@@ -1760,7 +1761,7 @@
 {
     memset(op_counts, 0, sizeof(op_counts));
     n_keyswitch = n_ntt = 0;
-    n_hops = n_decomp = 0, n_fold = 0;
+    n_hops = n_decomp = 0, n_fold = 0, n_rot_add = 0;
     t_bootstrap = 0.0;
     int i = (int)((header.hevm_header_size + config.config_body_length) / 8), j = 0;
     for (const WireOp &op : ops) {
@@ -2142,6 +2143,11 @@
     if (pairs) *pairs = V(vm)->n_fold;
 }
 
+void hevm_last_run_rot_add_stats(void *vm, int64_t *folded)
+{
+    if (folded) *folded = V(vm)->n_rot_add;
+}
+
 int64_t hevm_plan_lazy_groups(void *vm, int32_t *out, int64_t cap)
 {
     auto h = V(vm);
diff --git a/dacapo_amd/csrc/hevm_vm.hpp b/dacapo_amd/csrc/hevm_vm.hpp
--- a/dacapo_amd/csrc/hevm_vm.hpp
+++ b/dacapo_amd/csrc/hevm_vm.hpp
@@ -155,6 +155,7 @@
         std::vector<u32> elts;
         std::vector<const u64 *> keys;
         std::vector<int> ops;
+        bool add_fold = false;
         std::vector<int> plains;
     };
     struct Step {
@@ -165,6 +166,7 @@
         Handoff h;
         int fused_consumer = -1;
         bool fold_rs = false;
+        bool with_add = false;
         int gfirst = 0, gcount = 0;
         int unique = 0;
         std::vector<const u64 *> reads, writes;
@@ -207,6 +209,7 @@
         int64_t n_keyswitch = 0, n_ntt = 0;
         int64_t n_hops = 0, n_decomp = 0;
         int64_t n_fold = 0;
+        int64_t n_rot_add = 0;
         size_t launches = 0, max_live = 0;
         hipGraph_t graph = nullptr;
         hipGraphExec_t graph_exec = nullptr;
@@ -241,6 +244,7 @@
     bool ks_hoist = false;
     int ks_lazy = 0;
     bool ks_fold_rescale = false;
+    bool rot_add_fold = false;
     KsItem *d_hoist_items = nullptr;
     void rotate_hop_vm(CtView dst, CtView src, u32 elt, const u64 *key, int ell);
     bool chain_fusion = true;
@@ -258,6 +262,7 @@
     int64_t n_keyswitch = 0, n_ntt = 0;
     int64_t n_hops = 0, n_decomp = 0;
     int64_t n_fold = 0;
+    int64_t n_rot_add = 0;
     double t_bootstrap = 0.0;
 
     VmAllocs allocs;
diff --git a/dacapo_amd/csrc/options.cpp b/dacapo_amd/csrc/options.cpp
--- a/dacapo_amd/csrc/options.cpp
+++ b/dacapo_amd/csrc/options.cpp
@@ -37,6 +37,7 @@
     { "ks_hoist", 0 },
     { "ks_lazy_sum", 0 },
     { "ks_fold_rescale", 0 },
+    { "rot_add_fold", 1 },
     { "seal_compr", 0 },
     { "trace", 0 },
     { "step_profile", 0 },
@@ -59,6 +60,7 @@
     { "ks_fuse_mac_tiles", 1LL << 40 },
     { "sum_pair_min_wgs", 1024 },
     { "sum_group_min_wgs", 2048 },
+    { "rot_add_split_limbs", 160 },
 };
 
 static long long g_val[OPT_COUNT];
diff --git a/dacapo_amd/csrc/options.hpp b/dacapo_amd/csrc/options.hpp
--- a/dacapo_amd/csrc/options.hpp
+++ b/dacapo_amd/csrc/options.hpp
@@ -27,6 +27,7 @@
     OPT_KS_HOIST,
     OPT_KS_LAZY_SUM,
     OPT_KS_FOLD_RESCALE,
+    OPT_ROT_ADD_FOLD,
     OPT_SEAL_COMPR,
     OPT_TRACE,
     OPT_STEP_PROFILE,
@@ -49,6 +50,7 @@
     OPT_KS_FUSE_MAC_TILES,
     OPT_SUM_PAIR_MIN_WGS,
     OPT_SUM_GROUP_MIN_WGS,
+    OPT_ROT_ADD_SPLIT_LIMBS,
     OPT_COUNT
 };
 
diff --git a/dacapo_amd/csrc/plan.hpp b/dacapo_amd/csrc/plan.hpp
--- a/dacapo_amd/csrc/plan.hpp
+++ b/dacapo_amd/csrc/plan.hpp
@@ -10,6 +10,7 @@
     u32 elt;
     u32 slot;
     const u64 *plain = nullptr, *plain_sp = nullptr;
+    CtView add{ nullptr, 0 };
 };
 struct MulItem {
     CtView a, b, dst;
@@ -79,7 +80,8 @@
     u64 *tmp = nullptr;
 };
 
-void b_rotate_hops(Context &c, const BatchWs &w, const KsItem *d_items, int B, int ell, hipStream_t s, const Handoff &h = Handoff{}, int unique = 0);
+void b_rotate_hops(Context &c, const BatchWs &w, const KsItem *d_items, int B, int ell, hipStream_t s, const Handoff &h = Handoff{}, int unique = 0,
+                   bool with_add = false);
 void b_mul_relin(Context &c, const BatchWs &w, const MulItem *d_items, const u64 *relin_key, int B, int ell, hipStream_t s,
                  const Handoff &h = Handoff{});
 bool mul_relin_rescale_fused(const Context &c, int B, int ell);
diff --git a/dacapo_amd/csrc/plan_exec.hip b/dacapo_amd/csrc/plan_exec.hip
--- a/dacapo_amd/csrc/plan_exec.hip
+++ b/dacapo_amd/csrc/plan_exec.hip
@@ -49,7 +49,7 @@
     P.graph_exec = nullptr, P.graph = nullptr;
     P.vals.clear(), P.pops.clear(), P.steps.clear();
     P.n_keyswitch = P.n_ntt = 0;
-    P.n_hops = P.n_decomp = 0, P.n_fold = 0;
+    P.n_hops = P.n_decomp = 0, P.n_fold = 0, P.n_rot_add = 0;
     const size_t nreg = ciphers.size();
     const int S = streams;
     std::vector<int> cur(nreg, -1);
@@ -422,6 +422,43 @@
                 for (int pl : p.plains)
                     if (pl >= 0) need_sp.push_back(pl);
         ensure_special_limbs(need_sp);
+    }
+
+    if (rot_add_fold && !c.hybrid() && !ks_hoist) {
+        std::vector<int> wv(O.size(), 0);
+        auto wave_of_val = [&](int v) {
+            const int dp = V[(size_t)V[(size_t)v].root].def_pop;
+            return dp >= 0 ? wv[(size_t)dp] : 0;
+        };
+        bool any = false;
+        for (size_t si = 0; si < O.size(); si++) {
+            Pop &p = O[si];
+            if (p.dead) continue;
+            int w = 0;
+            for (int s : p.srcs) w = std::max(w, wave_of_val(s));
+            wv[si] = w + 1;
+            if (p.kind != P_SUM || p.srcs.size() != 2 || p.src_plain[0] >= 0 || p.src_plain[1] >= 0) continue;
+            const int dst = p.dst;
+            if (V[(size_t)dst].root != dst) continue;
+            for (int k = 0; k < 2; k++) {
+                const int rv = p.srcs[(size_t)k], av = p.srcs[(size_t)(1 - k)];
+                const Val &sv = V[(size_t)rv];
+                const int hi = sv.root == rv ? sv.def_pop : -1;
+                if (hi < 0) continue;
+                Pop &r = O[(size_t)hi];
+                if (r.kind != P_ROT || r.dead || !r.direct || r.rot != 1 || r.add_fold || r.dst != rv || r.level != p.level) continue;
+                if (sv.uses != 1 || sv.pinned || V[(size_t)dst].level != sv.level) continue;
+                if (V[(size_t)V[(size_t)av].root].def_pop >= hi || wave_of_val(av) >= wv[(size_t)hi]) continue;
+                r.srcs.push_back(av), r.add_fold = true;
+                r.dst = dst, V[(size_t)dst].def_pop = hi;
+                V[(size_t)rv].uses = 0, V[(size_t)rv].def_pop = -1;
+                p.dead = true, any = true;
+                break;
+            }
+        }
+        if (any)
+            for (size_t v = 0; v < V.size(); v++)
+                if (V[v].root != (int)v) V[v].def_pop = V[(size_t)V[v].root].def_pop;
     }
 
     int max_wave = 0;
@@ -772,6 +809,8 @@
                         if (hoisted && !slot_of.count(sv.p)) sources.push_back(KsItem{ sv, sv, nullptr, 1u, 0 });
                         const u32 slot = (c.hybrid() || hoisted) ? slot_of.emplace(sv.p, (u32)slot_of.size()).first->second : 0u;
                         h_ks.push_back(KsItem{ sv, view(O[(size_t)pi].dst, q), O[(size_t)pi].key, O[(size_t)pi].elt, slot });
+                        if (O[(size_t)pi].add_fold)
+                            h_ks.back().add = view(O[(size_t)pi].srcs[1], q), st.with_add = true, P.n_rot_add++;
                     }
                 st.unique = (int)slot_of.size();
                 st.gfirst = (int)h_ks.size(), st.gcount = (int)sources.size();
@@ -1166,6 +1205,8 @@
         for (auto &kv : ks)
             fprintf(stderr, "[dacapo_amd] plan:   %-8s level %2d: %5zu steps %6zu items\n", kn[kv.first.first], kv.first.second,
                     kv.second.first, kv.second.second);
+        fprintf(stderr, "[dacapo_amd] plan:   two-term sums added in their rotation's last kernel (option rot_add_fold): %lld items\n",
+                (long long)P.n_rot_add);
     }
     if (option(OPT_TRACE))
         fprintf(stderr, "[dacapo_amd] plan: %zu ops -> %zu pseudo-ops -> %zu steps (%zu on the auxiliary stream, %zu fused into their producer's last kernel) in %d waves, ~%zu launches, %zu live buffers (%.1f GB pool)\n",
@@ -1184,7 +1225,7 @@
             hoist_rotate_hops(c, w, P.d_ks + st.first, P.d_ks + st.gfirst, st.count, st.unique, st.level, q);
             break;
         }
-        b_rotate_hops(st.target < 0 ? *bctx : c, w, P.d_ks + st.first, st.count, st.level, q, st.h, st.unique); break;
+        b_rotate_hops(st.target < 0 ? *bctx : c, w, P.d_ks + st.first, st.count, st.level, q, st.h, st.unique, st.with_add); break;
     case P_ROTSUM:
         if (!c.hybrid()) {
             hoist_rotate_sum(c, w, P.d_ks + st.first, P.d_ks + st.gfirst + st.gcount, st.count, st.unique, P.d_ks + st.gfirst, st.gcount, st.level, q);
@@ -1422,7 +1463,7 @@
     for (const WireOp &op : ops)
         if (op.opcode <= 10) op_counts[op.opcode]++;
     n_keyswitch = P.n_keyswitch, n_ntt = P.n_ntt;
-    n_hops = P.n_hops, n_decomp = P.n_decomp, n_fold = P.n_fold;
+    n_hops = P.n_hops, n_decomp = P.n_decomp, n_fold = P.n_fold, n_rot_add = P.n_rot_add;
     t_bootstrap = 0.0;
     const long ps = (long)c.K * (long)c.N;
     if (plan_graph) {
diff --git a/dacapo_amd/lowlevel.py b/dacapo_amd/lowlevel.py
--- a/dacapo_amd/lowlevel.py
+++ b/dacapo_amd/lowlevel.py
@@ -73,6 +73,7 @@
         L.dc_ct_mul_relin.argtypes = [vp, u64p, lng, u64p, lng, u64p, lng, u64p, i32, vp]
         L.dc_ct_mul_relin_rescale.argtypes = [vp, u64p, lng, u64p, lng, u64p, lng, u64p, u64p, vp, i32, vp]
         L.dc_ct_rotate_hop.argtypes = [vp, u64p, lng, u64p, lng, C.c_uint32, u64p, i32, vp]
+        L.dc_ct_rotate_hop_add.argtypes = [vp, u64p, lng, u64p, lng, u64p, lng, C.c_uint32, u64p, i32, vp]
         L.dc_ct_rotate_hoisted.argtypes = [vp, vp, lng, u64p, lng, vp, vp, i32, i32, vp]
         L.dc_ct_rotate_sum_hoisted.argtypes = [vp, u64p, lng, vp, lng, vp, vp, vp, vp, i32, i32, vp]
         L.dc_ct_rescale.argtypes = [vp, u64p, lng, u64p, lng, i32, vp]
diff --git a/dacapo_amd/runner.py b/dacapo_amd/runner.py
--- a/dacapo_amd/runner.py
+++ b/dacapo_amd/runner.py
@@ -90,7 +90,8 @@
                                        ctypes.POINTER(ctypes.c_int64)]
     L.hevm_last_run_hoist_stats.argtypes = [ctypes.c_void_p, ctypes.POINTER(ctypes.c_int64), ctypes.POINTER(ctypes.c_int64)]
     L.hevm_last_run_fold_rescale_stats.argtypes = [ctypes.c_void_p, ctypes.POINTER(ctypes.c_int64)]
-    L.hevm_plan_lazy_groups.argtypes = [ctypes.c_void_p, ctypes.POINTER(ctypes.c_int32), ctypes.c_int64]
+    L.hevm_last_run_rot_add_stats.argtypes = [ctypes.c_void_p, ctypes.POINTER(ctypes.c_int64)]
+    L.hevm_plan_lazy_groups.argtypes =[ctypes.c_void_p, ctypes.POINTER(ctypes.c_int32), ctypes.c_int64]
     L.hevm_plan_lazy_groups.restype = ctypes.c_int64
     L.hevm_set_streams.argtypes = [ctypes.c_void_p, ctypes.c_int]
     L.hevm_select_stream.argtypes = [ctypes.c_void_p, ctypes.c_int]
@@ -363,8 +364,13 @@
         self.lw.hevm_last_run_fold_rescale_stats(self.vm, ctypes.byref(pairs))
         return pairs.value
 
+    def rot_add_stats(self):
+        folded = ctypes.c_int64()
+        self.lw.hevm_last_run_rot_add_stats(self.vm, ctypes.byref(folded))
+        return folded.value
+
     def stats(self):
-        counts = (ctypes.c_int64 * 11)()
+        counts =(ctypes.c_int64 * 11)()
         ks, ntt = ctypes.c_int64(), ctypes.c_int64()
         self.lw.hevm_last_run_stats(self.vm, counts, ctypes.byref(ks), ctypes.byref(ntt))
         return {"op_counts": list(counts), "keyswitches": ks.value, "ntts": ntt.value,
diff --git a/include/dacapo_ckks.h b/include/dacapo_ckks.h
--- a/include/dacapo_ckks.h
+++ b/include/dacapo_ckks.h
@@ -62,6 +62,8 @@
                              void *stream);
 void dc_ct_rotate_hop(dc_context *ctx, uint64_t *dst, long dst_stride, const uint64_t *src, long src_stride,
                       uint32_t galois_elt, const uint64_t *galois_key, int ell, void *stream);
+void dc_ct_rotate_hop_add(dc_context *ctx, uint64_t *dst, long dst_stride, const uint64_t *src, long src_stride, const uint64_t *add,
+                          long add_stride, uint32_t galois_elt, const uint64_t *galois_key, int ell, void *stream);
 void dc_ct_rotate_hoisted(dc_context *ctx, uint64_t *const *dsts, long dst_stride, const uint64_t *src, long src_stride,
                           const uint32_t *galois_elts, const uint64_t *const *galois_keys, int count, int ell, void *stream);
 void dc_ct_rotate_sum_hoisted(dc_context *ctx, uint64_t *dst, long dst_stride, const uint64_t *const *srcs, long src_stride,
diff --git a/include/hevm_abi.h b/include/hevm_abi.h
--- a/include/hevm_abi.h
+++ b/include/hevm_abi.h
@@ -60,6 +60,7 @@
 void hevm_last_run_stats(void *vm, int64_t *op_counts , int64_t *keyswitches, int64_t *ntts);
 void hevm_last_run_hoist_stats(void *vm, int64_t *hops, int64_t *decompositions);
 void hevm_last_run_fold_rescale_stats(void *vm, int64_t *pairs);
+void hevm_last_run_rot_add_stats(void *vm, int64_t *folded);
 int64_t hevm_plan_lazy_groups(void *vm, int32_t *out, int64_t cap);
 void hevm_set_streams(void *vm, int n);
 void hevm_select_stream(void *vm, int s);
```

Result: no change. 1.316 million NTT/s (-0.6%).
